# NBISweden/MrBayes

Hardware: AMD Instinct MI355X
Metric: site-pattern lnL (node-pattern conditional-likelihood) updates/sec (higher is better)
Workload: dtype f32

## Files before the change

### include/libhmsbeagle/beagle.h

```cpp
#ifndef MBAMD_LIBHMSBEAGLE_BEAGLE_H_
#define MBAMD_LIBHMSBEAGLE_BEAGLE_H_

#ifdef __cplusplus
extern "C" {
#endif

#define BEAGLE_DLLEXPORT __attribute__((visibility("default")))

enum BeagleReturnCodes {
    BEAGLE_SUCCESS                      =  0,
    BEAGLE_ERROR_GENERAL                = -1,
    BEAGLE_ERROR_OUT_OF_MEMORY          = -2,
    BEAGLE_ERROR_UNIDENTIFIED_EXCEPTION = -3,
    BEAGLE_ERROR_UNINITIALIZED_INSTANCE = -4,
    BEAGLE_ERROR_OUT_OF_RANGE           = -5,
    BEAGLE_ERROR_NO_RESOURCE            = -6,
    BEAGLE_ERROR_NO_IMPLEMENTATION      = -7,
    BEAGLE_ERROR_FLOATING_POINT         = -8
};

enum BeagleFlags {
    BEAGLE_FLAG_PRECISION_SINGLE    = 1 << 0,
    BEAGLE_FLAG_PRECISION_DOUBLE    = 1 << 1,
    BEAGLE_FLAG_COMPUTATION_SYNCH   = 1 << 2,
// ... 142 lines not shown
BEAGLE_DLLEXPORT int beagleWaitForPartials(int instance, const int* destinationPartials, int destinationPartialsCount);
BEAGLE_DLLEXPORT int beagleAccumulateScaleFactors(int instance, const int* scaleIndices, int count, int cumulativeScaleIndex);
BEAGLE_DLLEXPORT int beagleRemoveScaleFactors(int instance, const int* scaleIndices, int count, int cumulativeScaleIndex);
BEAGLE_DLLEXPORT int beagleResetScaleFactors(int instance, int cumulativeScaleIndex);
BEAGLE_DLLEXPORT int beagleCopyScaleFactors(int instance, int destScalingIndex, int srcScalingIndex);
BEAGLE_DLLEXPORT int beagleGetScaleFactors(int instance, int srcScalingIndex, double* outScaleFactors);

BEAGLE_DLLEXPORT int beagleCalculateRootLogLikelihoods(int instance, const int* bufferIndices,
                                                       const int* categoryWeightsIndices,
                                                       const int* stateFrequenciesIndices,
                                                       const int* cumulativeScaleIndices, int count,
                                                       double* outSumLogLikelihood);
BEAGLE_DLLEXPORT int beagleCalculateEdgeLogLikelihoods(int instance, const int* parentBufferIndices,
                                                       const int* childBufferIndices,
                                                       const int* probabilityIndices,
                                                       const int* firstDerivativeIndices,
                                                       const int* secondDerivativeIndices,
                                                       const int* categoryWeightsIndices,
                                                       const int* stateFrequenciesIndices,
                                                       const int* cumulativeScaleIndices, int count,
                                                       double* outSumLogLikelihood,
                                                       double* outSumFirstDerivative,
                                                       double* outSumSecondDerivative);
BEAGLE_DLLEXPORT int beagleGetSiteLogLikelihoods(int instance, double* outLogLikelihoods);
BEAGLE_DLLEXPORT int beagleGetSiteDerivatives(int instance, double* outFirstDerivatives, double* outSecondDerivatives);

BEAGLE_DLLEXPORT int beagleUpdatePrePartials(int instance, const BeagleOperation* operations, int operationCount,
                                             int cumulativeScaleIndex);
BEAGLE_DLLEXPORT int beagleSetDifferentialMatrix(int instance, int matrixIndex, const double* inMatrix);
BEAGLE_DLLEXPORT int beagleCalculateEdgeDerivatives(int instance, const int* postBufferIndices, const int* preBufferIndices,
                                                    const int* derivativeMatrixIndices, const int* categoryWeightsIndices,
                                                    int count, double* outDerivatives, double* outSumDerivatives,
                                                    double* outSumSquaredDerivatives);

BEAGLE_DLLEXPORT int beagleCalculateCrossProductDerivative(int instance, const int* postBufferIndices, const int* preBufferIndices,
                                                           const int* categoryRateIndices, const int* categoryWeightsIndices,
                                                           const double* edgeLengths, int count, double* outSumDerivatives,
                                                           double* outSumSquaredDerivatives);

BEAGLE_DLLEXPORT BeagleBenchmarkedResourceList* beagleGetBenchmarkedResourceList(
    int tipCount, int compactBufferCount, int stateCount, int patternCount, int categoryCount, int* resourceList,
    int resourceCount, long preferenceFlags, long requirementFlags, int eigenModelCount, int partitionCount,
    int calculateDerivatives, long benchmarkFlags);
BEAGLE_DLLEXPORT int beagleSetCPUThreadCount(int instance, int threadCount);
BEAGLE_DLLEXPORT int beagleSetPatternPartitions(int instance, int partitionCount, const int* inPatternPartitions);
BEAGLE_DLLEXPORT int beagleSetCategoryRatesWithIndex(int instance, int categoryRatesIndex, const double* inCategoryRates);
BEAGLE_DLLEXPORT int beagleUpdateTransitionMatricesWithMultipleModels(int instance, const int* eigenIndices,
                                                                      const int* categoryRateIndices,
                                                                      const int* probabilityIndices,
                                                                      const int* firstDerivativeIndices,
                                                                      const int* secondDerivativeIndices,
                                                                      const double* edgeLengths, int count);
BEAGLE_DLLEXPORT int beagleUpdatePartialsByPartition(int instance, const BeagleOperationByPartition* operations, int operationCount);
BEAGLE_DLLEXPORT int beagleAccumulateScaleFactorsByPartition(int instance, const int* scaleIndices, int count,
                                                             int cumulativeScaleIndex, int partitionIndex);
BEAGLE_DLLEXPORT int beagleRemoveScaleFactorsByPartition(int instance, const int* scaleIndices, int count,
                                                         int cumulativeScaleIndex, int partitionIndex);
BEAGLE_DLLEXPORT int beagleResetScaleFactorsByPartition(int instance, int cumulativeScaleIndex, int partitionIndex);
BEAGLE_DLLEXPORT int beagleCalculateRootLogLikelihoodsByPartition(int instance, const int* bufferIndices,
                                                                  const int* categoryWeightsIndices,
                                                                  const int* stateFrequenciesIndices,
                                                                  const int* cumulativeScaleIndices,
                                                                  const int* partitionIndices, int partitionCount, int count,
                                                                  double* outSumLogLikelihoodByPartition,
                                                                  double* outSumLogLikelihood);
BEAGLE_DLLEXPORT int beagleCalculateEdgeLogLikelihoodsByPartition(
    int instance, const int* parentBufferIndices, const int* childBufferIndices, const int* probabilityIndices,
    const int* firstDerivativeIndices, const int* secondDerivativeIndices, const int* categoryWeightsIndices,
    const int* stateFrequenciesIndices, const int* cumulativeScaleIndices, const int* partitionIndices, int partitionCount,
    int count, double* outSumLogLikelihoodByPartition, double* outSumLogLikelihood, double* outSumFirstDerivativeByPartition,
    double* outSumFirstDerivative, double* outSumSecondDerivativeByPartition, double* outSumSecondDerivative);

BEAGLE_DLLEXPORT int mbamdGetChildCount(int instance);
BEAGLE_DLLEXPORT int mbamdSynchronize(int instance);
BEAGLE_DLLEXPORT int mbamdGetScaleExponents(int instance, int srcScalingIndex, int* out);
BEAGLE_DLLEXPORT int mbamdSetRateMatrices(int instance, int firstEigenIndex, int count, const double* q, const double* pi, int mode);
BEAGLE_DLLEXPORT int mbamdSetRateMatricesFrom(int instance, int firstEigenIndex, int count, const double* q, const double* pi, int mode,
                                              int warmFirstEigenIndex);
BEAGLE_DLLEXPORT const char* mbamdGetLastError(void);
BEAGLE_DLLEXPORT int mbamdKernelTiming(int instance, int enable);
BEAGLE_DLLEXPORT int mbamdGetKernelTiming(int instance, double* outMilliseconds, long* outLaunches, int reset);
BEAGLE_DLLEXPORT int mbamdGetListCounts(int instance, long* out6);
BEAGLE_DLLEXPORT int mbamdGetWalkCounts(int instance, long* out2);
BEAGLE_DLLEXPORT int mbamdGetRecomputeCounts(int instance, long* out3);
BEAGLE_DLLEXPORT int mbamdGetSubtreeRecomputeCounts(int instance, long* out3);
BEAGLE_DLLEXPORT int mbamdGetStepTiming(int instance, double* outMilliseconds, long* outSteps, int reset);
BEAGLE_DLLEXPORT int mbamdSetKernelPath(int instance, int path);
BEAGLE_DLLEXPORT int mbamdSetDeferredResult(int instance, int enable);
BEAGLE_DLLEXPORT int mbamdWalkTrace(int instance, long long* out, int maxSteps, int* outSteps, int* outWaves);
BEAGLE_DLLEXPORT int mbamdFetchLogLikelihood(int instance, double* outSumLogLikelihood);
BEAGLE_DLLEXPORT int mbamdReduceLogLikelihood(int instance, double* deviceOut, void* waitingStream);
BEAGLE_DLLEXPORT int mbamdGetResourcePciBusId(int resource, char* out, int length);
BEAGLE_DLLEXPORT int mbamdGetInstanceDevices(int instance, int* outResources, int maxCount);

#ifdef __cplusplus
}
#endif
#endif
```

### mrbayes_amd/beagle.py

```python
from __future__ import annotations

import ctypes as C
import os
from typing import Optional, Sequence

import numpy as np

HERE = os.path.dirname(os.path.abspath(__file__))
DEFAULT_LIB = os.path.join(HERE, "libhmsbeagle.so")

BEAGLE_SUCCESS = 0
BEAGLE_ERROR_GENERAL = -1
BEAGLE_ERROR_OUT_OF_MEMORY = -2
BEAGLE_ERROR_UNINITIALIZED_INSTANCE = -4
BEAGLE_ERROR_OUT_OF_RANGE = -5
BEAGLE_ERROR_NO_RESOURCE = -6
BEAGLE_ERROR_NO_IMPLEMENTATION = -7
BEAGLE_ERROR_FLOATING_POINT = -8
BEAGLE_OP_NONE = -1

BEAGLE_FLAG_PRECISION_SINGLE = 1 << 0
BEAGLE_FLAG_PRECISION_DOUBLE = 1 << 1
BEAGLE_FLAG_EIGEN_REAL = 1 << 4
BEAGLE_FLAG_EIGEN_COMPLEX = 1 << 5
BEAGLE_FLAG_SCALING_ALWAYS = 1 << 8
BEAGLE_FLAG_SCALERS_LOG = 1 << 10
BEAGLE_FLAG_PROCESSOR_GPU = 1 << 16
BEAGLE_FLAG_SCALING_DYNAMIC = 1 << 25


class BeagleInstanceDetails(C.Structure):
    _fields_ = [("resourceNumber", C.c_int), ("resourceName", C.c_char_p), ("implName", C.c_char_p),
                ("implDescription", C.c_char_p), ("flags", C.c_long)]


class BeagleResource(C.Structure):
    _fields_ = [("name", C.c_char_p), ("description", C.c_char_p), ("supportFlags", C.c_long),
                ("requiredFlags", C.c_long)]


class BeagleResourceList(C.Structure):
    _fields_ = [("list", C.POINTER(BeagleResource)), ("length", C.c_int)]


class BeagleOperation(C.Structure):
    _fields_ = [("destinationPartials", C.c_int), ("destinationScaleWrite", C.c_int),
                ("destinationScaleRead", C.c_int), ("child1Partials", C.c_int),
                ("child1TransitionMatrix", C.c_int), ("child2Partials", C.c_int),
                ("child2TransitionMatrix", C.c_int)]


EXPORTS = [
    "beagleGetVersion", "beagleGetCitation", "beagleGetResourceList", "beagleCreateInstance",
    "beagleFinalizeInstance", "beagleFinalize", "beagleSetTipStates", "beagleSetTipPartials", "beagleSetPartials",
    "beagleGetPartials", "beagleSetEigenDecomposition", "beagleSetStateFrequencies", "beagleSetCategoryWeights",
    "beagleSetCategoryRates", "beagleSetPatternWeights", "beagleUpdateTransitionMatrices",
    "beagleSetTransitionMatrix", "beagleGetTransitionMatrix", "beagleConvolveTransitionMatrices", "beagleTransposeTransitionMatrices",
    "beagleSetTransitionMatrices", "beagleUpdatePartials", "beagleWaitForPartials",
    "beagleAccumulateScaleFactors", "beagleRemoveScaleFactors", "beagleResetScaleFactors", "beagleCopyScaleFactors",
    "beagleGetScaleFactors", "beagleCalculateRootLogLikelihoods", "beagleCalculateEdgeLogLikelihoods",
    "beagleGetSiteLogLikelihoods", "beagleGetSiteDerivatives", "beagleUpdatePrePartials", "beagleSetDifferentialMatrix",
    "beagleCalculateEdgeDerivatives", "beagleCalculateCrossProductDerivative", "mbamdSynchronize", "mbamdGetLastError", "mbamdKernelTiming",
    "mbamdGetKernelTiming", "mbamdGetListCounts", "mbamdGetWalkCounts", "mbamdGetRecomputeCounts", "mbamdGetSubtreeRecomputeCounts", "mbamdGetStepTiming", "mbamdUpdateFinalPartials", "mbamdGetScaledPartials", "mbamdSetKernelPath", "mbamdSetDeferredResult", "mbamdFetchLogLikelihood", "mbamdReduceLogLikelihood", "mbamdGetResourcePciBusId", "mbamdGetInstanceDevices",
    "mbamdGetScaleExponents", "mbamdGetChildCount", "mbamdSetRateMatrices", "mbamdSetRateMatricesFrom",
    "beagleGetBenchmarkedResourceList", "beagleSetCPUThreadCount", "beagleSetPatternPartitions",
    "beagleSetCategoryRatesWithIndex", "beagleUpdateTransitionMatricesWithMultipleModels", "beagleUpdatePartialsByPartition",
    "beagleAccumulateScaleFactorsByPartition", "beagleRemoveScaleFactorsByPartition", "beagleResetScaleFactorsByPartition",
    "beagleCalculateRootLogLikelihoodsByPartition", "beagleCalculateEdgeLogLikelihoodsByPartition",
]

_dp = C.POINTER(C.c_double)
_ip = C.POINTER(C.c_int)


class BeagleError(RuntimeError):
    def __init__(self, code: int, where: str, detail: str = ""):
        super().__init__("%s failed with code %d%s" % (where, code, (": " + detail) if detail else ""))
        self.code = code


def _d(a) -> np.ndarray:
    return np.ascontiguousarray(a, dtype=np.float64)


def _i(a) -> np.ndarray:
    return np.ascontiguousarray(a, dtype=np.int32)


def _opt_i(a) -> Optional[np.ndarray]:
    return None if a is None else _i(a)


def _ptr(a: Optional[np.ndarray]):
    return None if a is None else a.ctypes.data_as(_ip)


class BeagleLibrary:

    def __init__(self, path: Optional[str] = None):
        path = path or os.environ.get("MBAMD_LIBRARY") or DEFAULT_LIB
        if not os.path.exists(path):
            raise FileNotFoundError(
                "%s not found: build the HIP engine first (python -m mrbayes_amd.build). "
                "There is no CPU implementation to fall back to." % path)
        self.path = path
        self.lib = C.CDLL(path)
        for name in EXPORTS:
            if not hasattr(self.lib, name):
                raise AttributeError("%s does not export %s" % (path, name))
        L = self.lib
        L.beagleGetVersion.restype = C.c_char_p
        L.beagleGetCitation.restype = C.c_char_p
        L.mbamdGetLastError.restype = C.c_char_p
        L.beagleGetResourceList.restype = C.POINTER(BeagleResourceList)
        L.beagleCreateInstance.argtypes = [C.c_int] * 9 + [_ip, C.c_int, C.c_long, C.c_long,
                                                          C.POINTER(BeagleInstanceDetails)]
        L.beagleSetTipStates.argtypes = [C.c_int, C.c_int, _ip]
        L.beagleSetTipPartials.argtypes = [C.c_int, C.c_int, _dp]
        L.beagleSetPartials.argtypes = [C.c_int, C.c_int, _dp]
        L.beagleGetPartials.argtypes = [C.c_int, C.c_int, C.c_int, _dp]
        L.beagleSetEigenDecomposition.argtypes = [C.c_int, C.c_int, _dp, _dp, _dp]
        L.beagleSetStateFrequencies.argtypes = [C.c_int, C.c_int, _dp]
        L.beagleSetCategoryWeights.argtypes = [C.c_int, C.c_int, _dp]
        L.beagleSetCategoryRates.argtypes = [C.c_int, _dp]
        L.beagleSetPatternWeights.argtypes = [C.c_int, _dp]
        L.beagleUpdateTransitionMatrices.argtypes = [C.c_int, C.c_int, _ip, _ip, _ip, _dp, C.c_int]
        L.beagleSetTransitionMatrix.argtypes = [C.c_int, C.c_int, _dp, C.c_double]
        L.beagleGetTransitionMatrix.argtypes = [C.c_int, C.c_int, _dp]
        L.beagleConvolveTransitionMatrices.argtypes = [C.c_int, _ip, _ip, _ip, C.c_int]
        L.beagleTransposeTransitionMatrices.argtypes = [C.c_int, _ip, _ip, C.c_int]
        L.beagleSetTransitionMatrices.argtypes = [C.c_int, _ip, _dp, _dp, C.c_int]
        L.beagleUpdatePartials.argtypes = [C.c_int, C.POINTER(BeagleOperation), C.c_int, C.c_int]
        L.beagleWaitForPartials.argtypes = [C.c_int, _ip, C.c_int]
        L.beagleAccumulateScaleFactors.argtypes = [C.c_int, _ip, C.c_int, C.c_int]
        L.beagleRemoveScaleFactors.argtypes = [C.c_int, _ip, C.c_int, C.c_int]
        L.beagleResetScaleFactors.argtypes = [C.c_int, C.c_int]
        L.beagleCopyScaleFactors.argtypes = [C.c_int, C.c_int, C.c_int]
        L.beagleGetScaleFactors.argtypes = [C.c_int, C.c_int, _dp]
        L.beagleCalculateRootLogLikelihoods.argtypes = [C.c_int, _ip, _ip, _ip, _ip, C.c_int, _dp]
        L.beagleCalculateEdgeLogLikelihoods.argtypes = [C.c_int, _ip, _ip, _ip, _ip, _ip, _ip, _ip, _ip, C.c_int,
                                                        _dp, _dp, _dp]
        L.beagleGetSiteLogLikelihoods.argtypes = [C.c_int, _dp]
        L.beagleGetSiteDerivatives.argtypes = [C.c_int, _dp, _dp]
        L.beagleUpdatePrePartials.argtypes = [C.c_int, C.POINTER(BeagleOperation), C.c_int, C.c_int]
        L.beagleSetDifferentialMatrix.argtypes = [C.c_int, C.c_int, _dp]
        L.beagleCalculateEdgeDerivatives.argtypes = [C.c_int, _ip, _ip, _ip, _ip, C.c_int, _dp, _dp, _dp]
        L.beagleCalculateCrossProductDerivative.argtypes = [C.c_int, _ip, _ip, _ip, _ip, _dp, C.c_int, _dp, _dp]
        L.mbamdGetKernelTiming.argtypes = [C.c_int, _dp, C.POINTER(C.c_long), C.c_int]
        L.mbamdGetListCounts.argtypes = [C.c_int, C.POINTER(C.c_long)]
        L.mbamdGetWalkCounts.argtypes = [C.c_int, C.POINTER(C.c_long)]
        L.mbamdGetRecomputeCounts.argtypes = [C.c_int, C.POINTER(C.c_long)]
        L.mbamdGetSubtreeRecomputeCounts.argtypes = [C.c_int, C.POINTER(C.c_long)]
        L.mbamdGetStepTiming.argtypes = [C.c_int, _dp, C.POINTER(C.c_long), C.c_int]
        L.mbamdUpdateFinalPartials.argtypes = [C.c_int, C.c_void_p, C.c_int]
        L.mbamdGetScaledPartials.argtypes = [C.c_int, C.c_int, C.c_int, C.POINTER(C.c_float), C.POINTER(C.c_float)]
        L.mbamdFetchLogLikelihood.argtypes = [C.c_int, _dp]
        L.mbamdReduceLogLikelihood.argtypes = [C.c_int, C.c_void_p, C.c_void_p]
        L.mbamdGetResourcePciBusId.argtypes = [C.c_int, C.c_char_p, C.c_int]
        L.mbamdGetInstanceDevices.argtypes = [C.c_int, _ip, C.c_int]

    def version(self) -> str:
        return self.lib.beagleGetVersion().decode()

    def last_error(self) -> str:
        return self.lib.mbamdGetLastError().decode()

    def pci_bus_id(self, resource: int) -> str:
        buf = C.create_string_buffer(64)
        rc = self.lib.mbamdGetResourcePciBusId(resource, buf, 64)
        if rc != 0:
            raise BeagleError(rc, "mbamdGetResourcePciBusId", self.last_error())
        return buf.value.decode()

    def resources(self):
        rl = self.lib.beagleGetResourceList().contents
        return [(rl.list[i].name.decode(), rl.list[i].description.decode(), rl.list[i].supportFlags)
                for i in range(rl.length)]


_default: Optional[BeagleLibrary] = None


def library(path: Optional[str] = None) -> BeagleLibrary:
    global _default
    if path is not None:
        return BeagleLibrary(path)
    if _default is None:
        _default = BeagleLibrary()
    return _default


class BeagleInstance:

    def __init__(self, lib: BeagleLibrary, tip_count, partials_buffer_count, compact_buffer_count, state_count,
                 pattern_count, eigen_buffer_count, matrix_buffer_count, category_count, scale_buffer_count,
                 resource: Optional[int] = None, preference_flags=0, requirement_flags=0):
        self._L = lib
        self.lib = lib.lib
        self.details = BeagleInstanceDetails()
        rl = None
        rc = 0
        if resource is not None:
            arr = (C.c_int * 1)(resource)
            rl, rc = C.cast(arr, _ip), 1
        self.id = self.lib.beagleCreateInstance(tip_count, partials_buffer_count, compact_buffer_count, state_count,
                                                pattern_count, eigen_buffer_count, matrix_buffer_count,
                                                category_count, scale_buffer_count, rl, rc, preference_flags,
                                                requirement_flags, C.byref(self.details))
        if self.id < 0:
            raise BeagleError(self.id, "beagleCreateInstance", lib.last_error())
        self.state_count, self.pattern_count, self.category_count = state_count, pattern_count, category_count

    def _chk(self, code: int, where: str, allow=()):
        if code != BEAGLE_SUCCESS and code not in allow:
            raise BeagleError(code, where, self._L.last_error())
        return code

    def finalize(self):
        if self.id >= 0:
            self.lib.beagleFinalizeInstance(self.id)
            self.id = -1

    def __del__(self):
        try:
            self.finalize()
        except Exception:
            pass

    def set_tip_states(self, tip, states):
        a = _i(states)
        self._chk(self.lib.beagleSetTipStates(self.id, tip, a.ctypes.data_as(_ip)), "beagleSetTipStates")

    def set_tip_partials(self, tip, partials):
# ... 203 lines not shown
        self._chk(self.lib.beagleUpdateTransitionMatricesWithMultipleModels(
            self.id, g.ctypes.data_as(_ip), r.ctypes.data_as(_ip), p.ctypes.data_as(_ip), _ptr(d1), _ptr(d2), e.ctypes.data_as(_dp), len(p)),
            "beagleUpdateTransitionMatricesWithMultipleModels")

    def update_partials_by_partition(self, operations):
        a = _i(operations).reshape(-1, 9)
        self._chk(self.lib.beagleUpdatePartialsByPartition(self.id, a.ctypes.data_as(C.c_void_p), a.shape[0]),
                  "beagleUpdatePartialsByPartition")

    def reset_scale_factors_by_partition(self, cum, partition):
        self._chk(self.lib.beagleResetScaleFactorsByPartition(self.id, cum, partition), "beagleResetScaleFactorsByPartition")

    def accumulate_scale_factors_by_partition(self, idx, cum, partition):
        a = _i(idx)
        self._chk(self.lib.beagleAccumulateScaleFactorsByPartition(self.id, a.ctypes.data_as(_ip), len(a), cum, partition),
                  "beagleAccumulateScaleFactorsByPartition")

    def remove_scale_factors_by_partition(self, idx, cum, partition):
        a = _i(idx)
        self._chk(self.lib.beagleRemoveScaleFactorsByPartition(self.id, a.ctypes.data_as(_ip), len(a), cum, partition),
                  "beagleRemoveScaleFactorsByPartition")

    def calculate_edge_log_likelihoods_by_partition(self, parents, children, probs, weights, freqs, cums, partitions, count):
        p, ch, pr, w, f, c, pt = _i(parents), _i(children), _i(probs), _i(weights), _i(freqs), _i(cums), _i(partitions)
        by = np.zeros(len(pt))
        out = C.c_double(0.0)
        rc = self.lib.beagleCalculateEdgeLogLikelihoodsByPartition(
            self.id, p.ctypes.data_as(_ip), ch.ctypes.data_as(_ip), pr.ctypes.data_as(_ip), None, None, w.ctypes.data_as(_ip),
            f.ctypes.data_as(_ip), c.ctypes.data_as(_ip), pt.ctypes.data_as(_ip), len(pt), count, by.ctypes.data_as(_dp),
            C.byref(out), None, None, None, None)
        self._chk(rc, "beagleCalculateEdgeLogLikelihoodsByPartition", allow=(BEAGLE_ERROR_FLOATING_POINT,))
        return rc, by, out.value

    def calculate_edge_derivatives_by_partition(self, parents, children, probs, first, second, weights, freqs, cums, partitions):
        p, ch, pr, w, f, c, pt = _i(parents), _i(children), _i(probs), _i(weights), _i(freqs), _i(cums), _i(partitions)
        d1, d2 = _opt_i(first), _opt_i(second)
        by = [np.zeros(len(pt)) for _ in range(3)]
        tot = [C.c_double(0.0) for _ in range(3)]
        rc = self.lib.beagleCalculateEdgeLogLikelihoodsByPartition(
            self.id, p.ctypes.data_as(_ip), ch.ctypes.data_as(_ip), pr.ctypes.data_as(_ip), _ptr(d1), _ptr(d2), w.ctypes.data_as(_ip),
            f.ctypes.data_as(_ip), c.ctypes.data_as(_ip), pt.ctypes.data_as(_ip), len(pt), 1, by[0].ctypes.data_as(_dp), C.byref(tot[0]),
            by[1].ctypes.data_as(_dp) if d1 is not None else None, C.byref(tot[1]) if d1 is not None else None,
            by[2].ctypes.data_as(_dp) if d2 is not None else None, C.byref(tot[2]) if d2 is not None else None)
        self._chk(rc, "beagleCalculateEdgeLogLikelihoodsByPartition", allow=(BEAGLE_ERROR_FLOATING_POINT,))
        return (rc, (by[0], tot[0].value), (by[1], tot[1].value) if d1 is not None else None,
                (by[2], tot[2].value) if d2 is not None else None)

    def calculate_root_log_likelihoods_by_partition(self, buffers, weights, freqs, cums, partitions, count):
        b, w, f, c, pt = _i(buffers), _i(weights), _i(freqs), _i(cums), _i(partitions)
        by = np.zeros(len(pt))
        out = C.c_double(0.0)
        rc = self.lib.beagleCalculateRootLogLikelihoodsByPartition(
            self.id, b.ctypes.data_as(_ip), w.ctypes.data_as(_ip), f.ctypes.data_as(_ip), c.ctypes.data_as(_ip),
            pt.ctypes.data_as(_ip), len(pt), count, by.ctypes.data_as(_dp), C.byref(out))
        self._chk(rc, "beagleCalculateRootLogLikelihoodsByPartition", allow=(BEAGLE_ERROR_FLOATING_POINT,))
        return rc, by, out.value

    def get_site_log_likelihoods(self) -> np.ndarray:
        out = np.empty(self.pattern_count)
        self._chk(self.lib.beagleGetSiteLogLikelihoods(self.id, out.ctypes.data_as(_dp)), "beagleGetSiteLogLikelihoods")
        return out

    def synchronize(self):
        self._chk(self.lib.mbamdSynchronize(self.id), "mbamdSynchronize")

    def kernel_timing(self, enable: bool):
        self._chk(self.lib.mbamdKernelTiming(self.id, 1 if enable else 0), "mbamdKernelTiming")

    def get_kernel_timing(self, reset=True):
        ms, n = C.c_double(0.0), C.c_long(0)
        self._chk(self.lib.mbamdGetKernelTiming(self.id, C.byref(ms), C.byref(n), 1 if reset else 0), "mbamdGetKernelTiming")
        return ms.value, n.value

    def get_list_counts(self):
        out = (C.c_long * 6)()
        self._chk(self.lib.mbamdGetListCounts(self.id, out), "mbamdGetListCounts")
        return tuple(int(v) for v in out)

    def get_walk_counts(self):
        out = (C.c_long * 2)()
        self._chk(self.lib.mbamdGetWalkCounts(self.id, out), "mbamdGetWalkCounts")
        return tuple(int(v) for v in out)

    def get_recompute_counts(self):
        out = (C.c_long * 3)()
        self._chk(self.lib.mbamdGetRecomputeCounts(self.id, out), "mbamdGetRecomputeCounts")
        return tuple(int(v) for v in out)

    def get_subtree_recompute_counts(self):
        out = (C.c_long * 3)()
        self._chk(self.lib.mbamdGetSubtreeRecomputeCounts(self.id, out), "mbamdGetSubtreeRecomputeCounts")
        return tuple(int(v) for v in out)

    def update_final_partials(self, operations):
        a = _i(operations).reshape(-1, 5)
        self._chk(self.lib.mbamdUpdateFinalPartials(self.id, a.ctypes.data_as(C.c_void_p), a.shape[0]), "mbamdUpdateFinalPartials")

    def get_scaled_partials(self, idx, cumulative_scale_index=BEAGLE_OP_NONE):
        out = np.empty((self.category_count, self.pattern_count, self.state_count), dtype=np.float32)
        ln = np.empty(self.pattern_count, dtype=np.float32)
        self._chk(self.lib.mbamdGetScaledPartials(self.id, idx, cumulative_scale_index, out.ctypes.data_as(C.POINTER(C.c_float)),
                                                  ln.ctypes.data_as(C.POINTER(C.c_float))), "mbamdGetScaledPartials")
        return out, ln

    def get_step_timing(self, reset=True):
        ms, n = C.c_double(0.0), C.c_long(0)
        self._chk(self.lib.mbamdGetStepTiming(self.id, C.byref(ms), C.byref(n), 1 if reset else 0), "mbamdGetStepTiming")
        return ms.value, n.value

    def set_deferred_result(self, enable: bool):
        self._chk(self.lib.mbamdSetDeferredResult(self.id, 1 if enable else 0), "mbamdSetDeferredResult")

    def reduce_log_likelihood(self, device_ptr, waiting_stream=0):
        self._chk(self.lib.mbamdReduceLogLikelihood(self.id, C.c_void_p(device_ptr), C.c_void_p(waiting_stream)), "mbamdReduceLogLikelihood")

    def devices(self):
        out = (C.c_int * 64)()
        n = self.lib.mbamdGetInstanceDevices(self.id, C.cast(out, _ip), 64)
        return [int(out[i]) for i in range(min(n, 64))]

    def fetch_log_likelihood(self):
        out = C.c_double(0.0)
        rc = self.lib.mbamdFetchLogLikelihood(self.id, C.byref(out))
        self._chk(rc, "mbamdFetchLogLikelihood", allow=(BEAGLE_ERROR_FLOATING_POINT,))
        return rc, out.value
```

### mrbayes_amd/csrc/mbamd_engine.cpp

```cpp
#include <mutex>
#include <memory>

#include "mbamd_host.h"
#include "libhmsbeagle/mbamd_parsimony.h"
#include "mbamd_parsimony.h"
#include "mbamd_f32.h"
#include "mbamd_f64.h"

namespace mbamd {

static std::mutex g_mutex;

static BeagleResourceList g_resources = {nullptr, 0};
static std::vector<BeagleResource> g_resourceVec;
static std::vector<std::string> g_resourceNames, g_resourceDescs;
static const long kSupport = BEAGLE_FLAG_PRECISION_SINGLE | BEAGLE_FLAG_COMPUTATION_SYNCH | BEAGLE_FLAG_EIGEN_REAL |
                             BEAGLE_FLAG_SCALING_MANUAL | BEAGLE_FLAG_SCALING_ALWAYS | BEAGLE_FLAG_SCALING_DYNAMIC |
                             BEAGLE_FLAG_SCALERS_LOG | BEAGLE_FLAG_VECTOR_NONE | BEAGLE_FLAG_THREADING_NONE |
                             BEAGLE_FLAG_PROCESSOR_GPU | BEAGLE_FLAG_INVEVEC_STANDARD | BEAGLE_FLAG_FRAMEWORK_HIP;

static void buildResources()
{
    if (g_resources.list) return;
    int n = 0;
// ... 928 lines not shown
        if (crc) return crc;
        for (size_t e = 0; e < n; ++e) { sum[e] += part[e]; sq[e] += partSq[e]; }
        return BEAGLE_SUCCESS;
    });
    if (rc) return rc;
    if (outSumDerivatives) std::copy(sum.begin(), sum.end(), outSumDerivatives);
    if (outSumSquaredDerivatives) std::copy(sq.begin(), sq.end(), outSumSquaredDerivatives);
    return BEAGLE_SUCCESS;
}

int beagleCalculateCrossProductDerivative(int instance, const int* postBufferIndices, const int* preBufferIndices, const int* categoryRateIndices,
                                          const int* categoryWeightsIndices, const double* edgeLengths, int count, double* outSumDerivatives,
                                          double* outSumSquaredDerivatives)
{
    StatTimer st_(ST_LNL);
    GET_INSTANCE(instance);
    API_TRACE("beagleCalculateCrossProductDerivative(count=%d)", count);
    const char* const who = "beagleCalculateCrossProductDerivative";
    if (h->partitionCount > 1) return fail(BEAGLE_ERROR_NO_IMPLEMENTATION, who, "not on a multi-partition instance");
    if (outSumSquaredDerivatives) return fail(BEAGLE_ERROR_NO_IMPLEMENTATION, who, "outSumSquaredDerivatives must be NULL (a per-pattern square is an S x S matrix per pattern)");
    if (count < 0 || !outSumDerivatives ||
        (count > 0 && (!postBufferIndices || !preBufferIndices || !categoryRateIndices || !categoryWeightsIndices || !edgeLengths)))
        return fail(BEAGLE_ERROR_OUT_OF_RANGE, who, "null array");
    if (h->f64)
        return h->f64->crossProducts(postBufferIndices, preBufferIndices, categoryRateIndices, categoryWeightsIndices, edgeLengths, count, outSumDerivatives);
    const size_t SS = (size_t) h->dim.stateCount * h->dim.stateCount;
    std::vector<double> sum(SS, 0.0), part(SS);
    const int rc = each_engine(h, true, [&](Instance* c, const Handle::Span&) -> int {
        const int crc = c->crossProducts(postBufferIndices, preBufferIndices, categoryRateIndices, categoryWeightsIndices, edgeLengths, count, part.data());
        if (crc) return crc;
        for (size_t ij = 0; ij < SS; ++ij) sum[ij] += part[ij];
        return BEAGLE_SUCCESS;
    });
    if (rc) return rc;
    std::copy(sum.begin(), sum.end(), outSumDerivatives);
    return BEAGLE_SUCCESS;
}

int mbamdSynchronize(int instance)
{
    GET_INSTANCE(instance);
    return synchronize(h);
}
int mbamdKernelTiming(int instance, int enable)
{
    GET_INSTANCE(instance);
    if (h->f64) return BEAGLE_SUCCESS;
    EACH_ENGINE(false, (c->setTiming(enable != 0), BEAGLE_SUCCESS));
}
int mbamdGetKernelTiming(int instance, double* outMilliseconds, long* outLaunches, int reset)
{
    GET_INSTANCE(instance);
    double ms = 0.0;
    long launches = 0;
    const int rc = h->f64 ? h->f64->kernelTiming(&ms, &launches, reset) : each_engine(h, false, [&](Instance* c, const Handle::Span&) {
        double m = 0.0;
        const int trc = c->kernelTiming(&m, &launches, reset);
        ms = std::max(ms, m);
        return trc;
    });
    if (rc) return rc;
    if (outMilliseconds) *outMilliseconds = ms;
    if (outLaunches) *outLaunches = launches;
    return BEAGLE_SUCCESS;
}
int mbamdGetListCounts(int instance, long* out6)
{
    GET_INSTANCE(instance);
    if (!out6) return fail(BEAGLE_ERROR_OUT_OF_RANGE, "mbamdGetListCounts: null output");
    for (int i = 0; i < 6; ++i) out6[i] = 0;
    if (!in) return BEAGLE_SUCCESS;
    in->listCounts(out6);
    return BEAGLE_SUCCESS;
}
int mbamdGetWalkCounts(int instance, long* out2)
{
    GET_INSTANCE(instance);
    if (!out2) return fail(BEAGLE_ERROR_OUT_OF_RANGE, "mbamdGetWalkCounts: null output");
    out2[0] = out2[1] = 0;
    if (!in) return BEAGLE_SUCCESS;
    in->walkCounts(out2);
    return BEAGLE_SUCCESS;
}
int mbamdGetRecomputeCounts(int instance, long* out3)
{
    GET_INSTANCE_NOFLUSH(instance);
    if (!out3) return fail(BEAGLE_ERROR_OUT_OF_RANGE, "mbamdGetRecomputeCounts: null output");
    out3[0] = out3[1] = out3[2] = 0;
    if (h->f64) return BEAGLE_SUCCESS;
    EACH_ENGINE(false, (c->recomputeCounts(out3), BEAGLE_SUCCESS));
}
int mbamdGetSubtreeRecomputeCounts(int instance, long* out3)
{
    GET_INSTANCE_NOFLUSH(instance);
    if (!out3) return fail(BEAGLE_ERROR_OUT_OF_RANGE, "mbamdGetSubtreeRecomputeCounts: null output");
    out3[0] = out3[1] = out3[2] = 0;
    if (h->f64) return BEAGLE_SUCCESS;
    EACH_ENGINE(false, (c->subtreeRecomputeCounts(out3), BEAGLE_SUCCESS));
}
int mbamdGetStepTiming(int instance, double* outMilliseconds, long* outSteps, int reset)
{
    GET_INSTANCE(instance);
    if (h->f64) return fail(BEAGLE_ERROR_NO_IMPLEMENTATION, "mbamdGetStepTiming: not on a double-precision instance");
    double ms = 0.0;
    long steps = 0;
    const int rc = each_engine(h, false, [&](Instance* c, const Handle::Span&) {
        double m = 0.0;
        long st = 0;
        const int trc = c->stepTiming(&m, &st, reset);
        ms = std::max(ms, m);
        steps = std::max(steps, st);
        return trc;
    });
    if (rc) return rc;
    if (outMilliseconds) *outMilliseconds = ms;
    if (outSteps) *outSteps = steps;
    return BEAGLE_SUCCESS;
}
int mbamdSetKernelPath(int instance, int path)
{
    GET_INSTANCE(instance);
    if (h->f64) return BEAGLE_SUCCESS;
    if (path < 0 || path > 3) return fail(BEAGLE_ERROR_OUT_OF_RANGE, "mbamdSetKernelPath");
    return BEAGLE_SUCCESS;
}
int mbamdWalkTrace(int instance, long long* out, int maxSteps, int* outSteps, int* outWaves)
{
    GET_INSTANCE(instance);
    if (h->f64) return fail(BEAGLE_ERROR_NO_IMPLEMENTATION, "mbamdWalkTrace: not on a double-precision instance");
    if (!in) return fail(BEAGLE_ERROR_GENERAL, "set MBAMD_WALK_TRACE before creating the instance");
    return in->walkTrace(out, maxSteps, outSteps, outWaves);
}
int mbamdGetChildCount(int instance)
{
    GET_INSTANCE_NOFLUSH(instance);
    if (h->f64) return h->f64->childCount();
    return h->children.empty() ? 1 : (int) h->children.size();
}
int mbamdSetDeferredResult(int instance, int enable)
{
    GET_INSTANCE(instance);
    if (h->f64) return enable ? fail(BEAGLE_ERROR_NO_IMPLEMENTATION, "mbamdSetDeferredResult: not on a double-precision instance") : BEAGLE_SUCCESS;
    if (!in) return enable ? fail(BEAGLE_ERROR_NO_IMPLEMENTATION, "mbamdSetDeferredResult: not on a partitioned / sharded instance") : BEAGLE_SUCCESS;
    in->setDeferredResult(enable != 0);
    return BEAGLE_SUCCESS;
}
int mbamdReduceLogLikelihood(int instance, double* deviceOut, void* waitingStream)
{
    GET_INSTANCE(instance);
    if (!in) return fail(BEAGLE_ERROR_NO_IMPLEMENTATION, "mbamdReduceLogLikelihood: plain single-precision instances only");
    return in->reduceResult(deviceOut, waitingStream);
}
int mbamdGetResourcePciBusId(int resource, char* out, int length)
{
    if (out == nullptr || length < 2) return fail(BEAGLE_ERROR_OUT_OF_RANGE, "mbamdGetResourcePciBusId: buffer");
    int n = 0;
    if (hipGetDeviceCount(&n) != hipSuccess || resource < 0 || resource >= n) return fail(BEAGLE_ERROR_OUT_OF_RANGE, "mbamdGetResourcePciBusId: resource");
    HIP_TRY(hipDeviceGetPCIBusId(out, length, resource));
    return BEAGLE_SUCCESS;
}
int mbamdGetInstanceDevices(int instance, int* outResources, int maxCount)
{
    GET_INSTANCE_NOFLUSH(instance);
    if (h->children.empty()) { if (outResources && maxCount > 0) outResources[0] = h->device; return 1; }
    int n = 0;
    for (const Handle::Child& c : h->children) { if (outResources && n < maxCount) outResources[n] = c.in->device; ++n; }
// ... 142 lines not shown
```

### mrbayes_amd/csrc/mbamd_f32.h

```cpp
#ifndef MBAMD_F32_H_
#define MBAMD_F32_H_

#include <cmath>
#include <cstdlib>
#include <memory>
#include <unordered_map>

#include "mbamd_host.h"
#include "mbamd_kernels.h"
#include "mbamd_reports.h"
#include "libhmsbeagle/mbamd_reports.h"
#include "mbamd_walk4_host.h"
#include "mbamd_kernels_mfma.h"
#include "mbamd_derivatives.h"
#include "mbamd_preorder.h"
#include "mbamd_crossproducts.h"
#include "mbamd_matrix_products.h"

namespace mbamd {


static inline bool wg_compiled(int S) { return (S >= 2 && S <= 10 && S != 4) || S == 16 || S == 20 || S == 40 || (S >= 60 && S <= 63); }
#if !defined(MBAMD_WG_DEPTH61)
#define MBAMD_WG_DEPTH61 1
#endif
#define MBAMD_WG_DISPATCH(S, FN, ...)                                   \
    switch (S) {                                                        \
        case 2: FN<2, 8, 1, 2>(__VA_ARGS__); break;                     \
        case 3: FN<3, 8, 1, 2>(__VA_ARGS__); break;                     \
        case 5: FN<5, 8, 1, 2>(__VA_ARGS__); break;                     \
        case 6: FN<6, 8, 1, 2>(__VA_ARGS__); break;                     \
        case 7: FN<7, 8, 1, 2>(__VA_ARGS__); break;                     \
        case 8: FN<8, 8, 1, 2>(__VA_ARGS__); break;                     \
        case 9: FN<9, 8, 1, 2>(__VA_ARGS__); break;                     \
        case 10: FN<10, 8, 1, 2>(__VA_ARGS__); break;                   \
        case 16: FN<16, 8, 1, 2>(__VA_ARGS__); break;                   \
        case 20: FN<20, 8, 1, 2>(__VA_ARGS__); break;                   \
        case 40: FN<40, 4, 1, 1>(__VA_ARGS__); break;                   \
        case 60: FN<60, 4, 2, MBAMD_WG_DEPTH61>(__VA_ARGS__); break;    \
        case 61: FN<61, 4, 2, MBAMD_WG_DEPTH61>(__VA_ARGS__); break;    \
        case 62: FN<62, 4, 2, MBAMD_WG_DEPTH61>(__VA_ARGS__); break;    \
        default: FN<63, 4, 2, MBAMD_WG_DEPTH61>(__VA_ARGS__); break;    \
    }

template <int SC_, int WMAX_, int CH_, int DEPTH_>
static void raise_walkg_lds(int maxLds)
{
    if (hipFuncSetAttribute((const void*) k_walkg<SC_, WMAX_, CH_, DEPTH_>, hipFuncAttributeMaxDynamicSharedMemorySize, maxLds) != hipSuccess ||
        hipFuncSetAttribute((const void*) k_walkg<SC_, WMAX_, CH_, DEPTH_, WalkGArgsInline>, hipFuncAttributeMaxDynamicSharedMemorySize, maxLds) != hipSuccess)
        (void) hipGetLastError();
}

#define MBAMD_W4_UNSTORED_TIPS_DEFAULT 4
struct Walk4Recipe {
    int nops = 0;
    struct Op { int c1, c2, mode; bool in1, in2; } op[MBAMD_W4_UNSTORED_TIPS_MAX - 1];
    bool usesTip(int tip) const
    {
        for (int j = 0; j < nops; ++j) if ((!op[j].in1 && op[j].c1 == tip) || (!op[j].in2 && op[j].c2 == tip)) return true;
        return false;
    }
};

struct Plan {
    std::vector<int> key;
    uint64_t hash = 0, lastUse = 0;
    uint64_t lastLaunch = 0;
    PartialsOp* d_table = nullptr;
    size_t cap = 0;
    struct Segment {
        size_t first; int W, entries, nslots, tail = 2;
        bool plain = false, peel = false;
    };
    std::vector<Segment> segments;
    std::vector<Walk4Entry> inlineProg;
    struct Unstored { int entry, dst; Walk4Recipe r; int inner[MBAMD_W4_UNSTORED_TIPS_MAX - 2]; };
    std::vector<Unstored> unstoredSubtrees;
    size_t sideFirst = 0; int sideCount = 0;
    bool path = false;
    bool forked = false;
    bool pathG = false;
    int lists = 1;
    std::vector<int> start;
    bool anyScale = false;
    bool narrow = false;
    std::vector<std::pair<int, int>> chains;
    std::vector<std::pair<int, int>> spineChains;
    int tipTip = 0;
    int serialFrom = 0;
    std::vector<int> bufsRead, bufsWritten, scalesUsed;
};

struct PathStep {
    bool start, join;
    bool chainTip, sibTip;
    int arm;
    int dst, chain, sib;
    int mchain, msib;
    int scaleMode, scaleIdx;
};

struct Instance;
static int new_engine(std::unique_ptr<Instance>& out, const Dims& d, int patternCount, int dev, const Switches& sw);

struct Instance {
    Instance() = default;
    Instance(const Instance&) = delete;
    Instance& operator=(const Instance&) = delete;
    ~Instance();
    int device = 0;
    const char* implName() const;
    void printStats(int id) const;
    int synchronize() { HIP_TRY(hipStreamSynchronize(stream)); return BEAGLE_SUCCESS; }
    int setTipStates(int tip, const int* states);
    int importPartials(int idx, const double* in, bool hasCategories);
    int getPartials(int idx, double* out);
    int setPatternWeights(const double* w, int count) { return upload(d_pweights, w, sizeof(double) * count); }
    int setEigen(int idx, const double* U, const double* Ui, const double* lam);
    int setRateMatrices(int first, int count, const double* q, const double* pi, int mode, int warmFirst = -1);
    int setRates(int index, const double* r);
    int updateMatrices(int eigenIndex, const int* probIdx, const double* lengths, int count, int rateSet = 0,
                       const int* d1Idx = nullptr, const int* d2Idx = nullptr);
    int setMatrix(int idx, const double* in);
    int getMatrix(int idx, double* out);
    int convolveMatrices(const int* first, const int* second, const int* result, int count);
    int transposeMatrices(const int* input, const int* result, int count);
    int setMatrices(const int* idx, const double* in, int count);
    int updatePartials(const BeagleOperation* ops, int n, int cumIdx);
    int flushPending(bool keepPath = false);
    int resetScale(int idx, bool mayWait = false);
    int copyScale(int dst, int src);
    int accumulateScale(const int* idx, int n, int cumIdx, int sign, bool afterReset = false);
    int runDeferredReset() { const int idx = deferredReset; deferredReset = -1; return idx < 0 ? BEAGLE_SUCCESS : resetScale(idx); }
    int getScaleExponents(int idx, int* out);
    int integrate(const int* parent, const int* child, const int* prob, const int* wIdx, const int* fIdx,
                  const int* cumIdx, int count, double* out, bool launchOnly = false);
    int fetchResult(double* out);
    void setDeferredResult(bool on) { deferred = on; }
    int reduceResult(double* deviceOut, void* waitingStream);
    bool hasSites() const { return haveSite; }
    int getSites(double* out);
    int edgeDerivatives(int parent, int child, int prob, int d1, int d2, int wIdx, int fIdx, int cumIdx, double out3[3]);
    bool hasDerivatives() const { return derivValid; }
    const double* siteDerivatives(int order) const { return h_deriv + (size_t) order * Ppad; }
    int updatePrePartials(const BeagleOperation* ops, int n, int cumIdx);
    int edgeGradient(const int* post, const int* pre, const int* dmat, const int* wIdx, int count, double* sites, size_t siteStride,
                     double* sums, double* sumsSq);
    int crossProducts(const int* post, const int* pre, const int* rateIdx, const int* wIdx, const double* lengths, int count, double* out);
    int finalPass(const MbamdFinalOperation* ops, int count);
    int getScaledPartials(int idx, int cumIdx, float* out, float* outLn);
    void setTiming(bool on) { timing = on; }
    int kernelTiming(double* ms, long* launches, int reset);
    int stepTiming(double* ms, long* steps, int reset);
    void listCounts(long out6[6]) const { const long c[6] = {listsTotal, listsPath, forkedPaths, fusedPaths, listsWalked, opsWalked}; std::copy(c, c + 6, out6); }
    void walkCounts(long out2[2]) const { out2[0] = walksPlain; out2[1] = walksGeneric; }
    int walkTrace(long long* out, int maxSteps, int* outSteps, int* outWaves);
    void recomputeCounts(long out3[3]) const { out3[0] += leftUnstored; out3[1] += materialised; out3[2] += materialiseLaunches; }
    void subtreeRecomputeCounts(long out3[3]) const { out3[0] += leftUnstoredSub; out3[1] += materialisedSub; out3[2] += materialiseLaunchesSub; }

private:
    friend int new_engine(std::unique_ptr<Instance>&, const Dims&, int, int, const Switches&);
    hipStream_t stream{};
    int tipCount = 0, nBuffers = 0, S = 0, SP = 0, P = 0, Ppad = 0, nEigen = 0, nMatrices = 0, K = 0, nScale = 0;
    bool complexEigen = false;
    bool s4 = false;
    bool wg = false;
    bool noWalkG = false;
    bool arena() const { return s4 || wg; }
    bool mfma = false;
    int walkWaves = 1, lastWalkSteps = 0;
    Walk4Builder w4;
    std::unordered_map<uint64_t, Walk4Template> w4templates;
    uint64_t scheduleHits = 0, scheduleMisses = 0;
    std::vector<Walk4Op> w4ops;
    std::vector<int> w4key, w4writer, w4segList;
    std::vector<char> w4written, w4segRead, w4segWritten, w4segScale;
    std::vector<Walk4Entry> w4table;
    int8_t* arenaExp = nullptr;
    unsigned estride = 0;
    std::vector<int32_t*> wideScale;
    std::vector<char> scaleState;
    int lastWalkW = 0, lastWalkSlots = 0, lastWalkEntries = 0, lastWalkPhases = 0;
    bool walkCumFresh = false;
    typedef Walk4Recipe Recipe;
    std::vector<char> unstored;
    std::vector<Recipe> recipes;
    int nUnstored = 0;
    float* d_snap = nullptr;
    Plan* snapPlan = nullptr;
    void* d_storeProg = nullptr;     size_t storeProgCap = 0;
    std::vector<int> storeList;
    std::vector<Walk4Entry> storeProg;
    long leftUnstored = 0, materialised = 0, materialiseLaunches = 0;
    long leftUnstoredSub = 0, materialisedSub = 0, materialiseLaunchesSub = 0;
    int unstoredTips() const { return std::max(2, std::min(MBAMD_W4_UNSTORED_TIPS_MAX, sw.unstoredTips.value_or(MBAMD_W4_UNSTORED_TIPS_DEFAULT))); }
    std::vector<int> w4subTips, w4subOps, w4entryOf;
    int leaveUnstored(const Plan& plan);
    int flushSnapshot();
    int ensureStored(const int* bufs, int n);
    int ensureStoredSubtrees();
    int ensureStored(int a, int b = -1) { const int v[2] = {a, b}; return nUnstored ? ensureStored(v, 2) : BEAGLE_SUCCESS; }
    int storeUsersOfTip(int tip);
    void dropRecipe(int idx) { if (nUnstored && unstored[(size_t) idx]) { unstored[(size_t) idx] = 0; --nUnstored; } }
    std::vector<BeagleOperation> wgOps;
    std::vector<int> wgListStart, wgListCum;
    int32_t* wgCum[MBAMD_WG_MAXLISTS] = {nullptr, nullptr, nullptr, nullptr};
    int wgFresh = 0;
    uint8_t* arenaTipStates = nullptr;
    unsigned long wgTileBytes = 0;
    unsigned wgTipTileBytes = 0;
    size_t wgTabFloats = 0;
public:
    bool hasPending(bool path = true) const { return !pending.empty() || !wgListCum.empty() || (path && heldPath != nullptr); }
    bool hasWork(bool path = true) const { return hasPending(path) || !pendingJobs.empty(); }
private:
    Plan* heldPath = nullptr;
    int32_t* heldPathCum = nullptr;
    bool heldPathFresh = false;
    int heldPathDst = -1;
    int runHeldPath();
    int integratePath4(const int* child, const int* prob, const int* wIdx, const int* fIdx, const int* cumIdx);
    int updatePartialsG(const BeagleOperation* ops, int n, int cumIdx);
    int flushWalkG();
    int runWalkG(const Plan& plan);
    int checkOperation(const BeagleOperation& b, const std::vector<char>& written, const char*& what) const;
    std::vector<PathStep> pathSteps;
    bool recognisePath(const BeagleOperation* ops, int n, int L, bool& forked);
    Walk4Entry pathEntry(const PathStep& p, uint32_t pbuf, uint32_t tipb, uint32_t mbuf, int scratchRow) const;
    void pathPlan(Plan& plan, int entries, bool forked);
    bool buildPath4(Plan& plan, const BeagleOperation* ops, int n);
    bool buildPathG(Plan& plan, const BeagleOperation* ops, int n, const std::vector<int>& starts, int nl);
    Walk4Args walk4Args() const;
    WalkGArgs walkGArgs() const;
    int prepareCumulative(int idx, bool& fresh);
    void postResultFlag();
    bool scaleOpsIndependentOfPending(const int* idx, int n, int cumIdx) const;
    uint64_t launchClock = 0, syncedClock = 0;
    uint64_t flagClock = 0;
    uint32_t siteSeq = 0, seenSeq = 0;
    HostMirror h_freqs, h_weights;
    long long* d_trace = nullptr;

    int NT = 0, T = 0;
    size_t partialsFloats = 0, matrixFloats = 0, eigenDoubles = 0;

    std::vector<float*> partials;
    std::vector<uint8_t*> tipStates;
    std::vector<int32_t*> scale;
    std::vector<char> valid;
    float* arenaPartials = nullptr;
    uint64_t* arenaTips = nullptr;
    BlockGeom geom{64, 64, 64};
    float* matrices = nullptr;
    double *d_eigen = nullptr, *d_freqs = nullptr, *d_weights = nullptr, *d_rates = nullptr, *d_pweights = nullptr;
    double *d_site = nullptr;
    double* h_site = nullptr;
    double* h_site_dev = nullptr;
    bool siteToHost = false, siteOnHost = false;
    int nblocks = 0;
    double* h_deriv = nullptr;
    double* h_deriv_dev = nullptr;
    bool derivValid = false;
    std::vector<char> preOrder;
    void clearPreOrder(int idx) { if (idx >= 0 && idx < (int) preOrder.size()) preOrder[idx] = 0; }
    LnlOperands lastLnl;
// ... 69 lines not shown
    void armSums(bool launchOnly) { sumsArmed = !pendingResult && !deferred && !launchOnly && wait.arm(h_sums, (size_t) nblocks); }

    bool timing = false;
    std::vector<std::pair<hipEvent_t, hipEvent_t>> events;
    double timedMs = 0.0;
    long timedLaunches = 0, pendingLaunches = 0;
    hipEvent_t spanEv0{};
    bool spanOpen = false;
    std::vector<std::pair<hipEvent_t, hipEvent_t>> spans;
    double spanMs = 0.0;
    long spanCount = 0;
    int spanBegin()
    {
        if (!timing || spanOpen) return BEAGLE_SUCCESS;
        HIP_TRY(hipEventCreate(&spanEv0));
        HIP_TRY(hipEventRecord(spanEv0, stream));
        spanOpen = true;
        return BEAGLE_SUCCESS;
    }
    int spanEnd()
    {
        if (!spanOpen) return BEAGLE_SUCCESS;
        hipEvent_t e1{};
        HIP_TRY(hipEventCreate(&e1));
        HIP_TRY(hipEventRecord(e1, stream));
        spans.emplace_back(spanEv0, e1);
        spanOpen = false;
        if (spans.size() > 4096) {
            HIP_TRY(hipStreamSynchronize(stream));
            spanFold();
        }
        return BEAGLE_SUCCESS;
    }
    int spanFold()
    {
        for (auto& ev : spans) {
            float t = 0.0f;
            if (hipEventElapsedTime(&t, ev.first, ev.second) == hipSuccess) { spanMs += t; ++spanCount; }
            (void) hipEventDestroy(ev.first);
            (void) hipEventDestroy(ev.second);
        }
        spans.clear();
        return BEAGLE_SUCCESS;
    }
    int launchesBegin(hipEvent_t& ev0, hipEvent_t& ev1)
    {
        { int src = spanBegin(); if (src) return src; }
        if (!timing) return BEAGLE_SUCCESS;
        HIP_TRY(hipEventCreate(&ev0));
        HIP_TRY(hipEventCreate(&ev1));
        HIP_TRY(hipEventRecord(ev0, stream));
        return BEAGLE_SUCCESS;
    }
    int launchesEnd(hipEvent_t ev0, hipEvent_t ev1)
    {
        if (!timing) return BEAGLE_SUCCESS;
        HIP_TRY(hipEventRecord(ev1, stream));
        events.emplace_back(ev0, ev1);
        return BEAGLE_SUCCESS;
    }
    int eventsFold()
    {
        for (auto& ev : events) {
            float t = 0.0f;
            HIP_TRY(hipEventElapsedTime(&t, ev.first, ev.second));
            timedMs += t;
            (void) hipEventDestroy(ev.first);
            (void) hipEventDestroy(ev.second);
        }
        events.clear();
        return BEAGLE_SUCCESS;
    }

    bool deferred = false, pendingResult = false;
    hipEvent_t reduceEvent{};
    std::vector<int32_t*> finalExpOf;
    std::unordered_map<int, int32_t*> finalExpOwn;

    std::vector<std::pair<Plan*, int>> pending;
    std::vector<Plan*> plans;
    uint64_t planClock = 0;
    int layoutEpoch = 0;
    long planHits = 0, planMisses = 0, fusedPaths = 0, heldPaths = 0, forkedPaths = 0, listsTotal = 0, listsPath = 0, opsWalked = 0, listsWalked = 0;
    long walksPlain = 0, walksGeneric = 0;

    int grow(void** p, size_t* cap, size_t bytes) { return grow_device(stream, p, cap, bytes, std::max(bytes, *cap * 2)); }

    int upload(void* dst, const void* src, size_t bytes)
    {
        if (bytes == 0) return BEAGLE_SUCCESS;
        if (bytes > stage.capacity() / 2) {
            HIP_TRY(hipStreamSynchronize(stream));
            HIP_TRY(hipMemcpy(dst, src, bytes, hipMemcpyHostToDevice));
            return BEAGLE_SUCCESS;
        }
        if (bytes <= ((size_t) 256 << 10) && bytes % 4 == 0 && (reinterpret_cast<uintptr_t>(dst) & 3u) == 0) return ringCopy(dst, src, bytes);
        size_t off = 0;
        int rc = stage.put(src, bytes, stream, &off);
        if (rc) return rc;
        HIP_TRY(hipMemcpyAsync(dst, stage.host(off), bytes, hipMemcpyHostToDevice, stream));
        return BEAGLE_SUCCESS;
    }
    int ringCopy(void* dst, const void* src, size_t bytes);

public:
    int setFreqs(int idx, const double* f) { return h_freqs.send((size_t) nEigen * S, (size_t) idx * S, f, (size_t) S, [&] { return upload(d_freqs + (size_t) idx * S, f, sizeof(double) * S); }); }
    int setWeights(int idx, const double* w) { return h_weights.send((size_t) nEigen * K, (size_t) idx * K, w, (size_t) K, [&] { return upload(d_weights + (size_t) idx * K, w, sizeof(double) * K); }); }
private:

    int stageDirect(const void* src, size_t bytes, const void** devPtr)
    {
        if (((bytes + 63) & ~(size_t) 63) > stage.capacity() / 2) return fail(BEAGLE_ERROR_OUT_OF_MEMORY, "staging ring too small");
        size_t off = 0;
        int rc = stage.put(src, bytes, stream, &off);
        if (rc) return rc;
        *devPtr = stage.dev(off);
        return BEAGLE_SUCCESS;
    }

    int ensurePartials(int idx)
    {
        if (partials[idx]) return BEAGLE_SUCCESS;
        if (arena()) return fail(BEAGLE_ERROR_GENERAL, "partials arena not initialised");
        float* p = nullptr;
        HIP_TRY(hipMalloc(&p, partialsFloats * sizeof(float)));
        HIP_TRY(hipMemsetAsync(p, 0, partialsFloats * sizeof(float), stream));
        partials[idx] = p;
        return BEAGLE_SUCCESS;
    }
    int ensureScale(int idx)
    {
        if (scale[idx]) return BEAGLE_SUCCESS;
        if (arena()) return fail(BEAGLE_ERROR_GENERAL, "exponent arena not initialised");
        int32_t* p = nullptr;
        HIP_TRY(hipMalloc(&p, (size_t) Ppad * sizeof(int32_t)));
        HIP_TRY(hipMemsetAsync(p, 0, (size_t) Ppad * sizeof(int32_t), stream));
        scale[idx] = p;
        return BEAGLE_SUCCESS;
    }
    float* matrixPtr(int idx) const { return matrices + (size_t) idx * matrixFloats; }

    int create(const Dims& dim, int patternCount, int dev, const Switches& switches);

    int configureWalk();
    void wgGeometry(int lists, int& W, int& slots) const;
    int setTipMasks(int tip, const std::vector<uint8_t>& masks);
    std::vector<int> eigenWarm;
    std::vector<char> eigenShield;
    int updatePartials4(const BeagleOperation* ops, int n, int cumIdx);
    int buildWalk(Plan& plan, const BeagleOperation* ops, int n, const int* listOf = nullptr, bool perList = false);
    int ensureWide(int idx);
    int accumulate4(const int* idx, int n, int cumIdx, int sign);
    int deferredReset = -1;
    int checkIntegrate(const int* parent, const int* child, const int* prob, const int* wIdx, const int* fIdx, const int* cumIdx, int count);
    int integrate4(const int* parent, const int* child, const int* prob, const int* wIdx, const int* fIdx,
                   const int* cumIdx, int count);
    int integrateLevels(const int* parent, const int* child, const int* prob, const int* wIdx, const int* fIdx,
                        const int* cumIdx, int count);
    int buildGeneric(Plan& plan, std::vector<PartialsOp>& dev, const std::vector<int>& dstIdx, const std::vector<int>& c1Idx,
                     const std::vector<int>& c2Idx);
    int runWalk(const Plan& plan, int32_t* cum);
    int runGeneric(const Plan& plan, int32_t* cum);
    Plan* cachedPlan(const int* key, size_t nints, bool& build);
    int planBuilt(Plan& plan, int rc);
    int planTable(Plan& plan, const void* table, size_t bytes);
    int timedRun(const Plan& plan, int32_t* cum);
// ... 122 lines not shown
        wgTileBytes = (unsigned long) (nBuffers + 1) * K * tb;
        wgTipTileBytes = (unsigned) nBuffers * MBAMD_WG_TW;
        estride = (unsigned) (scale.size() + MBAMD_WG_SCRATCH_ROWS) * K * 64;
        const size_t pBytes = nt * wgTileBytes, tBytes = nt * wgTipTileBytes, eBytes = nb * (size_t) estride;
        HIP_TRY(hipMalloc(&arenaPartials, pBytes));
        HIP_TRY(hipMalloc(&arenaTipStates, tBytes));
        HIP_TRY(hipMalloc(&arenaExp, eBytes));
        HIP_TRY(hipMemsetAsync(arenaPartials, 0, pBytes, stream));
        HIP_TRY(hipMemsetAsync(arenaTipStates, S, tBytes, stream));
        HIP_TRY(hipMemsetAsync(arenaExp, 0, eBytes, stream));
        wideScale.assign(scale.size(), nullptr);
        scaleState.assign(scale.size(), 0);
        if (sw.verbose)
            std::fprintf(stderr, "[mbamd] arenas: partials +%zu, tips +%zu, exponents +%zu bytes\n", pBytes, tBytes, eBytes);
        for (int i = 0; i < nBuffers; ++i) partials[i] = arenaPartials + (size_t) i * K * tb / 4;
    }

    HIP_TRY(hipMalloc(&matrices, std::max<size_t>(1, (size_t) nMatrices * matrixFloats) * sizeof(float)));
    HIP_TRY(hipMemsetAsync(matrices, 0, std::max<size_t>(1, (size_t) nMatrices * matrixFloats) * sizeof(float), stream));
    if (wg && nMatrices > 0) {
        const int total = nMatrices * K * S;
        MBAMD_LAUNCH(k_wg_init_tables, (unsigned) ((total + 255) / 256), 256, 0, stream, matrices, matrixFloats, wgTabFloats, S, K, total);
        HIP_TRY(hipGetLastError());
    }
    HIP_TRY(hipMalloc(&d_eigen, std::max<size_t>(1, (size_t) nEigen * eigenDoubles) * sizeof(double)));
    if (complexEigen) HIP_TRY(hipMemsetAsync(d_eigen, 0, std::max<size_t>(1, (size_t) nEigen * eigenDoubles) * sizeof(double), stream));
    HIP_TRY(hipMalloc(&d_freqs, std::max<size_t>(1, (size_t) nEigen * S) * sizeof(double)));
    HIP_TRY(hipMalloc(&d_weights, std::max<size_t>(1, (size_t) nEigen * K) * sizeof(double)));
    HIP_TRY(hipMalloc(&d_rates, (size_t) K * sizeof(double)));
    HIP_TRY(hipMalloc(&d_pweights, (size_t) Ppad * sizeof(double)));
    HIP_TRY(hipMalloc(&d_site, (size_t) Ppad * sizeof(double)));
    nblocks = Ppad / 64;
    if (!s4 && S >= 8) nblocks = Ppad / 32;
    if (wg) nblocks = Ppad / MBAMD_INTEGRATE_WG_PATTERNS;
    HIP_TRY(hipHostMalloc(&h_sums, (size_t) nblocks * sizeof(double), hipHostMallocDefault));
    HIP_TRY(hipHostGetDevicePointer((void**) &h_sums_dev, h_sums, 0));
    wait.create(!sw.noPoll);
    { int rc = stage.create((size_t) 8 << 20, 64); if (rc) return rc; }

    std::vector<double> ones(std::max(Ppad, K), 1.0);
    HIP_TRY(hipMemcpy(d_rates, ones.data(), (size_t) K * sizeof(double), hipMemcpyHostToDevice));
    std::vector<double> pw(Ppad, 0.0);
    std::fill(pw.begin(), pw.begin() + P, 1.0);
    HIP_TRY(hipMemcpy(d_pweights, pw.data(), (size_t) Ppad * sizeof(double), hipMemcpyHostToDevice));
    std::vector<double> w((size_t) std::max(1, nEigen) * K, 1.0 / K);
    HIP_TRY(hipMemcpy(d_weights, w.data(), (size_t) nEigen * K * sizeof(double), hipMemcpyHostToDevice));
    HIP_TRY(hipStreamSynchronize(stream));
    return BEAGLE_SUCCESS;
}

inline Instance::~Instance()
{
    (void) hipSetDevice(device);
    (void) hipStreamSynchronize(stream);
    if (arena()) {
        void* arenas[] = {arenaPartials, arenaTips, arenaTipStates, arenaExp};
        for (void* a : arenas) if (a) (void) hipFree(a);
        for (int32_t* w : wideScale) if (w) (void) hipFree(w);
    } else {
        for (float* p : partials) if (p) (void) hipFree(p);
        for (uint8_t* p : tipStates) if (p) (void) hipFree(p);
        for (int32_t* p : scale) if (p) (void) hipFree(p);
    }
    pending.clear();
    wgOps.clear(); wgListStart.clear(); wgListCum.clear();
    for (Plan* pl : plans) { if (pl->d_table) (void) hipFree(pl->d_table); delete pl; }
    plans.clear();
    void* bufs[] = {matrices, d_eigen, d_freqs, d_weights, d_rates, d_pweights, d_site,
                    d_ev, d_tmp, d_trace, d_q, d_preTable, d_snap, d_storeProg};
    for (void* b : bufs) if (b) (void) hipFree(b);
    if (h_sums) (void) hipHostFree(h_sums);
    wait.destroy();
    if (h_site) (void) hipHostFree(h_site);
    if (h_deriv) (void) hipHostFree(h_deriv);
    stage.destroy();
    for (auto& ev : events) { (void) hipEventDestroy(ev.first); (void) hipEventDestroy(ev.second); }
    for (auto& ev : spans) { (void) hipEventDestroy(ev.first); (void) hipEventDestroy(ev.second); }
    if (spanOpen) (void) hipEventDestroy(spanEv0);
    if (reduceEvent) (void) hipEventDestroy(reduceEvent);
    for (auto& kv : finalExpOwn) if (kv.second) (void) hipFree(kv.second);
    (void) hipStreamDestroy(stream);
}

inline int Instance::configureWalk()
{
    int numCU = 256;
    hipDeviceProp_t prop;
    if (hipGetDeviceProperties(&prop, device) == hipSuccess && prop.multiProcessorCount > 0) numCU = prop.multiProcessorCount;
    const int maxLds = 160 * 1024;
    if (s4 && (hipFuncSetAttribute((const void*) k_walk4_t<Walk4Args>, hipFuncAttributeMaxDynamicSharedMemorySize, maxLds) != hipSuccess ||
               hipFuncSetAttribute((const void*) k_walk4_t<Walk4Args, true>, hipFuncAttributeMaxDynamicSharedMemorySize, maxLds) != hipSuccess ||
               hipFuncSetAttribute((const void*) k_walk4_t<Walk4ArgsInline>, hipFuncAttributeMaxDynamicSharedMemorySize, maxLds) != hipSuccess))
        (void) hipGetLastError();
    if (wg) {
        const unsigned slotBytes = wg_block_bytes(S);
        MBAMD_WG_DISPATCH(S, raise_walkg_lds, maxLds);
        wgGeometry(1, w4.maxW, w4.maxSlots);
        w4.maxSlots1 = w4.maxSlots;
        if (!sw.walkWaves && !sw.maxLdsSlots) {
            const long wgsG = (long) (Ppad / MBAMD_WG_TW) * K;
            const int perCUG = (int) std::max(1L, (wgsG + numCU - 1) / numCU);
            w4.maxSlots1 = std::max(w4.maxSlots, std::min(24, (int) (((160 * 1024) / std::min(perCUG, 32) - 64 - MBAMD_WG_STAGE) / (int) slotBytes)));
        }
        w4.memSlots = false;
        w4.leadNops = MBAMD_WG_LEAD; w4.unroll = 3; w4.tailNops = MBAMD_WG_TAIL;
        w4.prefetchDistance = 0;
        if (sw.walkSmallPhase) w4.smallPhase = std::max(1, *sw.walkSmallPhase);
        if (sw.verbose) std::fprintf(stderr, "[mbamd] tree walk (%d states): %ld workgroups, up to %d waves x %d slots of %u bytes\n",
                                     S, (long) (Ppad / MBAMD_WG_TW) * K, w4.maxW, w4.maxSlots, slotBytes);
        return BEAGLE_SUCCESS;
    }
    const long wgs = (long) (Ppad / 64) * K;
    const int perCU = (int) std::max(1L, (wgs + numCU - 1) / numCU);
    const int ldsPerWG = (160 * 1024) / std::min(perCU, 32) - 64;
    auto slotsFor = [&](int W) { return (ldsPerWG / W - MBAMD_W4_STAGE) / 1024; };
    int W = (int) std::max(1L, std::min((long) MBAMD_W4_MAXW, (14L * numCU + wgs / 2) / wgs));
    while (W > 1 && slotsFor(W) < 7) --W;
    if (sw.walkWaves) W = std::max(1, std::min(MBAMD_W4_MAXW, *sw.walkWaves));
    int slots = std::max(3, std::min(48, slotsFor(W)));
    if (sw.maxLdsSlots) slots = std::max(3, std::min(150 / W, *sw.maxLdsSlots));
    w4.maxW = W;
    w4.maxSlots = slots;
    w4.maxSlots1 = sw.maxLdsSlots ? slots : std::max(slots, std::min(40, slotsFor(1)));
    if (sw.walkPrefetch) w4.prefetchDistance = std::max(0, *sw.walkPrefetch);
    w4.forward = true;
    w4.safeWaits = sw.walkSafe;
    if (sw.walkSmallPhase) w4.smallPhase = std::max(1, *sw.walkSmallPhase);
    if (sw.verbose) std::fprintf(stderr, "[mbamd] tree walk: %ld workgroups (%d per CU), up to %d waves x %d slots\n", wgs, perCU, W, slots);
    return BEAGLE_SUCCESS;
}

inline void Instance::wgGeometry(int lists, int& W, int& slots) const
{
    int numCU = 256;
    hipDeviceProp_t prop;
    if (hipGetDeviceProperties(&prop, device) == hipSuccess && prop.multiProcessorCount > 0) numCU = prop.multiProcessorCount;
    const int maxW = S > 32 ? 4 : 8, wavesPerCU = S > 32 ? 6 : 12;
    const int slotBytes = (int) wg_block_bytes(S);
    const long wgs = (long) (Ppad / MBAMD_WG_TW) * K * lists;
    const int perCU = (int) std::max(1L, (wgs + numCU - 1) / numCU);
    const int ldsPerWG = (160 * 1024) / std::min(perCU, 32) - 64;
    auto slotsFor = [&](int w) { return (ldsPerWG / w - MBAMD_WG_STAGE) / slotBytes; };
    long want = std::max(1L, std::min((long) maxW, ((long) wavesPerCU * numCU + wgs / 2) / wgs));
    W = 1;
    while (W * 2 <= want) W *= 2;
    while (W > 1 && slotsFor(W) < 4) W /= 2;
    if (sw.walkWaves) W = std::max(1, std::min(maxW, *sw.walkWaves));
    slots = std::max(3, std::min(24, slotsFor(W)));
    if (sw.maxLdsSlots) slots = std::max(1, std::min((160 * 1024 / W - MBAMD_WG_STAGE) / slotBytes, *sw.maxLdsSlots));
}

inline int Instance::setTipMasks(int tip, const std::vector<uint8_t>& h)
{
    const size_t nb = (size_t) Ppad / 64;
    std::vector<uint64_t> planes(nb * 4, 0);
    for (int c = 0; c < Ppad; ++c)
        for (int i = 0; i < 4; ++i)
            if (h[c] >> i & 1u) planes[(size_t) (c >> 6) * 4 + i] |= (uint64_t) 1 << (c & 63);
    if (nUnstored) {
        const int src = storeUsersOfTip(tip);
        if (src) return src;
        dropRecipe(tip);
    }
    HIP_TRY(hipStreamSynchronize(stream));
    HIP_TRY(hipMemcpy2D(arenaTips + (size_t) tip * 4, (size_t) geom.tstride * 8, planes.data(), 32, 32, nb, hipMemcpyHostToDevice));
    if (!tipStates[tip]) layoutEpoch++;
    tipStates[tip] = reinterpret_cast<uint8_t*>(arenaTips + (size_t) tip * 4);
    return BEAGLE_SUCCESS;
}

inline int Instance::setTipStates(int tip, const int* states)
{
    if (tip < 0 || tip >= nBuffers) return fail(BEAGLE_ERROR_OUT_OF_RANGE, "beagleSetTipStates: tip index");
    clearPreOrder(tip);
    std::vector<uint8_t> h(Ppad, (uint8_t) S);
    for (int c = 0; c < P; ++c) h[c] = (uint8_t) ((states[c] < 0 || states[c] >= S) ? S : states[c]);
    if (s4) {
        for (int c = 0; c < Ppad; ++c) h[c] = (uint8_t) (h[c] >= 4 ? 0xF : 1u << h[c]);
        return setTipMasks(tip, h);
    }
    if (wg) {
        HIP_TRY(hipStreamSynchronize(stream));
        HIP_TRY(hipMemcpy2D(arenaTipStates + (size_t) tip * MBAMD_WG_TW, (size_t) wgTipTileBytes, h.data(), MBAMD_WG_TW, MBAMD_WG_TW, (size_t) Ppad / MBAMD_WG_TW, hipMemcpyHostToDevice));
        if (!tipStates[tip]) layoutEpoch++;
        tipStates[tip] = arenaTipStates + (size_t) tip * MBAMD_WG_TW;
        return BEAGLE_SUCCESS;
    }
    if (!tipStates[tip]) { HIP_TRY(hipMalloc(&tipStates[tip], (size_t) Ppad)); layoutEpoch++; }
    return upload(tipStates[tip], h.data(), (size_t) Ppad);
}

inline int Instance::importPartials(int idx, const double* in, bool hasCategories)
{
    if (idx < 0 || idx >= nBuffers) return fail(BEAGLE_ERROR_OUT_OF_RANGE, "partials buffer index");
    if (idx < (int) finalExpOf.size()) finalExpOf[idx] = nullptr;
    clearPreOrder(idx);
    if (s4 && !hasCategories) {
        std::vector<uint8_t> h(Ppad, 0xF);
        bool binary = true;
        for (int c = 0; c < P && binary; ++c) {
            unsigned m = 0;
            for (int i = 0; i < 4; ++i) {
                const double v = in[(size_t) c * 4 + i];
                if (v == 1.0) m |= 1u << i;
                else if (v != 0.0) binary = false;
            }
            h[c] = (uint8_t) m;
        }
        if (binary) return setTipMasks(idx, h);
    }
// ... 672 lines not shown
    scaleState[idx] = 2;
    return BEAGLE_SUCCESS;
}

inline int Instance::updatePartials4(const BeagleOperation* ops, int n, int cumIdx)
{
    if (heldPath) { int prc = runHeldPath(); if (prc) return prc; }
    if (snapPlan) { int src = flushSnapshot(); if (src) return src; }
    if (nUnstored) {
        std::vector<int>& ext = w4segList;
        std::vector<char>& written = w4written;
        ext.clear();
        written.assign((size_t) nBuffers, 0);
        for (int o = 0; o < n; ++o) {
            for (const int c : {ops[o].child1Partials, ops[o].child2Partials})
                if (c >= 0 && c < nBuffers && unstored[(size_t) c] && !written[(size_t) c]) ext.push_back(c);
            if (ops[o].destinationPartials >= 0 && ops[o].destinationPartials < nBuffers) written[(size_t) ops[o].destinationPartials] = 1;
        }
        if (!ext.empty()) { int src = ensureStored(ext.data(), (int) ext.size()); if (src) return src; }
    }
    int32_t* cumPtr = nullptr;
    walkCumFresh = false;
    if (cumIdx != BEAGLE_OP_NONE) {
        int rc = prepareCumulative(cumIdx, walkCumFresh);
        if (rc) return rc;
        cumPtr = wideScale[cumIdx];
    }
    bool build;
    Plan* plan = cachedPlan(reinterpret_cast<const int*>(ops), (size_t) n * 7, build);
    if (build) {
        int rc = flushMatrices();
        if (rc == BEAGLE_SUCCESS) {
            StatTimer st_(ST_PLAN);
            plan->path = plan->forked = false;
            plan->unstoredSubtrees.clear();
            rc = buildPath4(*plan, ops, n) ? BEAGLE_SUCCESS : buildWalk(*plan, ops, n);
        }
        if (planBuilt(*plan, rc)) return rc;
    }
    for (int o = 0; o < n; ++o) {
        valid[ops[o].destinationPartials] = 1;
        dropRecipe(ops[o].destinationPartials);
        if (ops[o].destinationScaleWrite != BEAGLE_OP_NONE) scaleState[ops[o].destinationScaleWrite] = 1;
    }
    int mrc = flushMatrices();
    if (mrc) return mrc;
    listsTotal++;
    if (plan->path) { listsPath++; if (plan->forked) forkedPaths++; }
    else { listsWalked++; opsWalked += n; }
    if (plan->path && !sw.noFusePath && K <= 8 && plan->inlineProg.size() <= MBAMD_W4_INLINE) {
        heldPath = plan;
        heldPaths++;
        heldPathCum = cumPtr;
        heldPathFresh = walkCumFresh;
        heldPathDst = ops[n - 1].destinationPartials;
        return BEAGLE_SUCCESS;
    }
    return timedRun(*plan, cumPtr);
}

inline int Instance::buildWalk(Plan& plan, const BeagleOperation* ops, int n, const int* listOf, bool perList)
{
    const int scratchScale = (int) scale.size();
    std::vector<int>& segList = w4segList;
    segList.clear();
    std::vector<char>& written = w4written;
    written.assign((size_t) nBuffers, 0);
    w4table.clear();
    plan.segments.clear();
    plan.unstoredSubtrees.clear();
    std::vector<Walk4Op>& seg = w4ops;
    seg.clear();
    std::vector<char>&segRead = w4segRead, &segWritten = w4segWritten, &segScale = w4segScale;
    segRead.assign((size_t) nBuffers, 0); segWritten.assign((size_t) nBuffers, 0); segScale.assign(scale.size() + 1, 0);
    if (w4writer.size() < (size_t) nBuffers) w4writer.assign((size_t) nBuffers, -1);
    int reloads = 0, externals = 0, phases = 0;
    auto flushSegment = [&]() -> int {
        if (seg.empty()) return BEAGLE_SUCCESS;
        std::vector<int>& key = w4key;
        key.clear();
        key.reserve(seg.size() * 3 + 4);
        key.push_back((int) seg.size()); key.push_back(w4.maxW); key.push_back(w4.maxSlots + 256 * w4.maxSlots1);
        key.push_back(w4.prefetchDistance * 2 + (w4.safeWaits ? 1 : 0));
        {
            std::vector<int>& writer = w4writer;
            constexpr int RO = MBAMD_W4_UNSTORED_TIPS_MAX - 1;
            w4subTips.assign(wg ? 0 : seg.size(), 0);
            w4subOps.assign(wg ? 0 : seg.size() * RO, -1);
            for (size_t o = 0; o < seg.size() && !wg; ++o) {
                const Walk4Op& op = seg[o];
                const int w1 = op.tip1 ? -1 : writer[op.c1], w2 = op.tip2 ? -1 : writer[op.c2];
                const int t1 = op.tip1 ? 1 : (w1 >= 0 ? w4subTips[(size_t) w1] : 0), t2 = op.tip2 ? 1 : (w2 >= 0 ? w4subTips[(size_t) w2] : 0);
                if (t1 && t2 && t1 + t2 <= MBAMD_W4_UNSTORED_TIPS_MAX && (op.tip1 || op.tip2 || op.c1 != op.c2)) {
                    w4subTips[o] = t1 + t2;
                    int below = 0, *mine = &w4subOps[o * RO];
                    for (const int w : {std::min(w1, w2), std::max(w1, w2)})
                        for (int j = 0; w >= 0 && j < RO && w4subOps[(size_t) w * RO + j] >= 0; ++j) mine[below++] = w4subOps[(size_t) w * RO + j];
                    mine[below] = (int) o;
                }
                writer[op.dst] = (int) o;
            }
            for (size_t o = 0; o < seg.size() && !wg; ++o) writer[seg[o].dst] = -1;
            for (size_t o = 0; o < seg.size(); ++o) {
                key.push_back(seg[o].tip1 ? -1 : writer[seg[o].c1]);
                key.push_back(seg[o].tip2 ? -1 : writer[seg[o].c2]);
                key.push_back((int) seg[o].tip1 | ((int) seg[o].tip2 << 1) | ((!seg[o].tip1 && !seg[o].tip2 && seg[o].c1 == seg[o].c2) ? 4 : 0) |
                              ((seg[o].scaleWrite < 0 && seg[o].scaleRead >= 0) ? 8 : 0));
                writer[seg[o].dst] = (int) o;
            }
            for (size_t o = 0; o < seg.size(); ++o) writer[seg[o].dst] = -1;
        }
        const uint64_t kh = fnv1a(key.data(), key.size());
        auto it = w4templates.find(kh);
        if (it == w4templates.end() || it->second.key != key) {
            scheduleMisses++;
            if (w4templates.size() >= 8192) w4templates.clear();
            Walk4Template& t = w4templates[kh];
            bool ok = w4.build(seg, t);
            if (!ok) {
                Walk4Builder plain = w4;
                plain.prefetchDistance = 0;
                ok = plain.build(seg, t);
                if (!ok) { plain.maxW = 1; ok = plain.build(seg, t); }
            }
            if (!ok) { w4templates.erase(kh); return fail(BEAGLE_ERROR_GENERAL, "tree-walk scheduler: cannot place this list"); }
            t.key = key;
            it = w4templates.find(kh);
        } else {
            scheduleHits++;
        }
        const Walk4Template& t = it->second;
        reloads += t.reloads; externals += t.externals; phases = std::max(phases, t.phases);
        Plan::Segment sg;
        sg.first = w4table.size();
        sg.W = t.W; sg.entries = t.entries; sg.nslots = t.nslots; sg.tail = t.tail;
        sg.plain = t.plain && !wg; sg.peel = t.peel;
        plan.segments.push_back(sg);
        w4table.resize(sg.first + t.prog.size());
        const uint32_t slotb = wg ? wg_block_bytes(S) : 1024u;
        const uint32_t pbuf = wg ? (uint32_t) K * slotb : (uint32_t) ((size_t) (Ppad / 64) * K);
        const uint32_t ebuf = (uint32_t) K * 64u, mbuf = wg ? (uint32_t) (matrixFloats * 4) : (uint32_t) K * 64u;
        int prevKept = -1;
        w4entryOf.assign(seg.size(), -1);
        for (size_t i = 0; i < t.prog.size(); ++i) {
            const Walk4Template::Entry& te = t.prog[i];
            Walk4Entry& e = w4table[sg.first + i];
            std::memset(&e, 0, sizeof e);
            if (i % (size_t) t.entries == 0) prevKept = -1;
            uint32_t flags = te.flags, mode = SCALE_NONE, keep = 0;
            e.ewrite = (uint32_t) scratchScale * ebuf;
            e.eread = (uint32_t) scratchScale * ebuf;
            e.ewrite = (uint32_t) (scratchScale + (int) (i % (size_t) (wg ? MBAMD_WG_SCRATCH_ROWS : MBAMD_W4_SCRATCH_ROWS))) * ebuf;
            if (wg) {
                e.dst = (uint32_t) nBuffers * pbuf;
                if (te.op >= 0) {
                    const Walk4Op& op = seg[te.op];
                    e.dst = (uint32_t) op.dst * pbuf;
                    if (op.tip1) { e.c1 = (uint32_t) op.c1 * (uint32_t) MBAMD_WG_TW; flags |= MBAMD_W4_TIP1; }
                    else if (te.c1slot == 0xFF) { e.c1 = (uint32_t) op.c1 * pbuf; flags |= MBAMD_WG_MEM1; }
                    else e.c1 = (uint32_t) te.c1slot * slotb;
                    if (op.tip2) { e.c2 = (uint32_t) op.c2 * (uint32_t) MBAMD_WG_TW; flags |= MBAMD_W4_TIP2; }
                    else if (te.c2slot == 0xFF) { e.c2 = (uint32_t) op.c2 * pbuf; flags |= MBAMD_WG_MEM2; }
                    else e.c2 = (uint32_t) te.c2slot * slotb;
                    e.m1 = (uint32_t) op.m1 * mbuf;
                    e.m2 = (uint32_t) op.m2 * mbuf;
                    if (te.dslot != 0xFF) { keep = te.dslot; flags |= MBAMD_W4_KEEP; }
                    if (!op.tip1 && te.c1slot != 0xFF && (int) te.c1slot == prevKept) flags |= MBAMD_WG_PREV1;
                    if (!op.tip2 && te.c2slot != 0xFF && (int) te.c2slot == prevKept) flags |= MBAMD_WG_PREV2;
                    prevKept = te.dslot != 0xFF ? (int) te.dslot : -1;
                    mode = op.scaleWrite >= 0 ? SCALE_WRITE : (op.scaleRead >= 0 ? SCALE_READ : SCALE_NONE);
                    if (op.scaleWrite >= 0) e.ewrite = (uint32_t) op.scaleWrite * ebuf;
                    if (op.scaleRead >= 0) e.eread = (uint32_t) op.scaleRead * ebuf;
                    e.ctl = flags | (mode << 8) | ((uint32_t) segList[te.op] << 10) | (keep << 16);
                } else {
                    e.ctl = (flags & (MBAMD_W4_NOP | MBAMD_W4_BARRIER)) | MBAMD_W4_NOP;
                }
                continue;
            }
            if (te.pfOp[0] >= 0) {
                const Walk4Op& p0 = seg[te.pfOp[0]];
                e.dst = (uint32_t) (te.pfChild[0] == 0 ? p0.c1 : p0.c2) * pbuf;
                e.c1 = (uint32_t) te.pfSlot[0] * 1024u;
                flags |= MBAMD_W4_PF0 | MBAMD_W4_NOP;
                if (te.pfOp[1] >= 0) {
                    const Walk4Op& p1 = seg[te.pfOp[1]];
                    e.c2 = (uint32_t) (te.pfChild[1] == 0 ? p1.c1 : p1.c2) * pbuf;
                    e.m1 = (uint32_t) te.pfSlot[1] * 1024u;
                    flags |= MBAMD_W4_PF1;
                }
            } else if (te.op >= 0) {
                const Walk4Op& op = seg[te.op];
                e.dst = (uint32_t) op.dst * pbuf;
                if (op.tip1) { e.c1 = (uint32_t) op.c1 * 32u; flags |= MBAMD_W4_TIP1; }
                else if (te.c1slot == 0xFE) flags |= MBAMD_W4_FWD1;
                else e.c1 = (uint32_t) te.c1slot * 1024u;
                if (op.tip2) { e.c2 = (uint32_t) op.c2 * 32u; flags |= MBAMD_W4_TIP2; }
                else if (te.c2slot == 0xFE) flags |= MBAMD_W4_FWD2;
                else e.c2 = (uint32_t) te.c2slot * 1024u;
                e.m1 = (uint32_t) op.m1 * mbuf;
                e.m2 = (uint32_t) op.m2 * mbuf;
                if (te.dslot != 0xFF) { keep = te.dslot; flags |= MBAMD_W4_KEEP; }
                mode = op.scaleWrite >= 0 ? SCALE_WRITE : (op.scaleRead >= 0 ? SCALE_READ : SCALE_NONE);
                if (op.scaleWrite >= 0) e.ewrite = (uint32_t) op.scaleWrite * ebuf;
                if (op.scaleRead >= 0) e.eread = (uint32_t) op.scaleRead * ebuf;
                w4entryOf[(size_t) te.op] = (int) (sg.first + i);
                const int subTips = w4subTips[(size_t) te.op];
                if (sg.plain && t.W == 1 && subTips >= 2 && subTips <= unstoredTips()) {
                    constexpr int RO = MBAMD_W4_UNSTORED_TIPS_MAX - 1;
                    const int* const sub = &w4subOps[(size_t) te.op * RO];
                    Plan::Unstored u;
                    u.entry = (int) (sg.first + i); u.dst = op.dst;
                    for (int& x : u.inner) x = -1;
                    bool placed = true;
                    for (int j = 0; j < RO && sub[j] >= 0; ++j) {
                        const Walk4Op& so = seg[(size_t) sub[j]];
                        Walk4Recipe::Op& ro = u.r.op[u.r.nops++];
                        ro.mode = so.scaleWrite >= 0 ? SCALE_WRITE : (so.scaleRead >= 0 ? SCALE_READ : SCALE_NONE);
                        ro.in1 = !so.tip1; ro.in2 = !so.tip2;
                        ro.c1 = so.c1; ro.c2 = so.c2;
                        for (int q = 0; q < j; ++q) {
                            if (ro.in1 && seg[(size_t) sub[q]].dst == so.c1) ro.c1 = q;
                            if (ro.in2 && seg[(size_t) sub[q]].dst == so.c2) ro.c2 = q;
                        }
                        if (sub[j] != te.op) { u.inner[j] = w4entryOf[(size_t) sub[j]]; placed = placed && u.inner[j] >= 0; }
                    }
                    if (placed) plan.unstoredSubtrees.push_back(u);
                }
            }
            if (te.vmwait != 0xFF) flags |= MBAMD_W4_VMWAIT;
            if ((i + 1) % (size_t) t.entries != 0) {
                const Walk4Template::Entry& tn = t.prog[i + 1];
                if (tn.op >= 0 && seg[tn.op].scaleWrite < 0 && seg[tn.op].scaleRead >= 0) flags |= MBAMD_W4_NEXT_READS;
            }
            e.ctl = flags | (mode << 8) | ((uint32_t) (te.vmwait == 0xFF ? 0 : te.vmwait) << 10) | (keep << 16);
            if (sg.plain) {
                if (te.op >= 0) e.ctl |= walk4_kind_of(flags);
                e.eread = (flags & MBAMD_W4_TIP1) ? e.c1 : 0u;
            }
        }
        lastWalkW = t.W; lastWalkSlots = t.nslots; lastWalkEntries = t.entries; lastWalkPhases = t.phases;
        seg.clear();
        segList.clear();
        std::fill(segRead.begin(), segRead.end(), 0);
        std::fill(segWritten.begin(), segWritten.end(), 0);
        std::fill(segScale.begin(), segScale.end(), 0);
        return BEAGLE_SUCCESS;
    };
    for (int o = 0; o < n; ++o) {
        const BeagleOperation& b = ops[o];
        const char* what;
        if (const int crc = checkOperation(b, written, what)) return fail(crc, what);
        Walk4Op w;
        w.dst = b.destinationPartials;
        w.c1 = b.child1Partials; w.c2 = b.child2Partials;
        w.m1 = b.child1TransitionMatrix; w.m2 = b.child2TransitionMatrix;
        const uint8_t tip[2] = {(uint8_t) (tipStates[w.c1] && !written[w.c1]), (uint8_t) (tipStates[w.c2] && !written[w.c2])};
        w.tip1 = tip[0]; w.tip2 = tip[1];
        w.scaleWrite = w.scaleRead = -1;
        if (b.destinationScaleWrite != BEAGLE_OP_NONE) {
            w.scaleWrite = b.destinationScaleWrite;
        } else if (b.destinationScaleRead != BEAGLE_OP_NONE) {
            if (scaleState[b.destinationScaleRead] == 2 && !segScale[b.destinationScaleRead])
                return fail(BEAGLE_ERROR_NO_IMPLEMENTATION, "beagleUpdatePartials: destinationScaleRead names a cumulative buffer");
            w.scaleRead = b.destinationScaleRead;
        }
        bool hazard = segWritten[w.dst] || segRead[w.dst];
        if (perList && o > 0 && listOf[o] != listOf[o - 1]) hazard = true;
        if (w.scaleWrite >= 0 && segScale[w.scaleWrite]) hazard = true;
        if (w.scaleRead >= 0 && segScale[w.scaleRead] == 2) hazard = true;
        if (hazard) {
            int rc = flushSegment();
            if (rc) return rc;
        }
        segWritten[w.dst] = 1;
        if (!tip[0]) segRead[w.c1] = 1;
        if (!tip[1]) segRead[w.c2] = 1;
        if (w.scaleWrite >= 0) segScale[w.scaleWrite] = 2;
        if (w.scaleRead >= 0 && !segScale[w.scaleRead]) segScale[w.scaleRead] = 1;
        written[w.dst] = 1;
        seg.push_back(w);
        segList.push_back(listOf ? listOf[o] : 0);
    }
    int rc = flushSegment();
    if (rc) return rc;
    if (sw.verbose)
        std::fprintf(stderr, "[mbamd] walk plan: %d ops, %zu segment(s), W=%d, %d entries/wave, %d slots/wave, %d phases, %d reloads, %d external children\n",
                     n, plan.segments.size(), lastWalkW, lastWalkEntries, lastWalkSlots, phases, reloads, externals);
    plan.inlineProg.clear();
    const bool inlineForm = !sw.noInlinePrograms && plan.segments.size() == 1 && w4table.size() <= (size_t) MBAMD_W4_INLINE;
    plan.sideFirst = 0; plan.sideCount = 0;
    if (s4 && !sw.storeTipPairs && !sw.noPlainWalk && !inlineForm && plan.segments.size() == 1 && plan.segments[0].plain) {
        for (const Plan::Unstored& u : plan.unstoredSubtrees) w4table[(size_t) u.entry].ctl |= MBAMD_W4_NOSTORE;
        plan.sideFirst = w4table.size();
        for (const Plan::Unstored& u : plan.unstoredSubtrees) {
            if (u.r.nops < 2) continue;
            Walk4Entry side;
            std::memset(&side, 0, sizeof side);
            side.ctl = (uint32_t) u.entry; side.dst = (uint32_t) (u.r.nops - 1);
            side.c1 = (uint32_t) u.inner[0]; side.c2 = (uint32_t) (u.r.nops > 2 ? u.inner[1] : u.inner[0]);
            w4table.push_back(side);
            plan.sideCount++;
        }
    } else {
        plan.unstoredSubtrees.clear();
    }
    if (inlineForm) {
        plan.inlineProg = w4table;
        return BEAGLE_SUCCESS;
    }
    return planTable(plan, w4table.data(), w4table.size() * sizeof(Walk4Entry));
}

inline int Instance::ringCopy(void* dst, const void* src, size_t bytes)
{
    const void* ring = nullptr;
    int rc = stageDirect(src, bytes, &ring);
    if (rc) return rc;
    if (bytes % 16 == 0 && (reinterpret_cast<uintptr_t>(dst) & 15u) == 0) {
        const unsigned n16 = (unsigned) (bytes / 16);
        MBAMD_LAUNCH(k_copy_from_ring, (n16 + 255u) / 256u, 256, 0, stream, static_cast<const copy16_t*>(ring), static_cast<copy16_t*>(dst), n16);
    } else {
        const unsigned n4 = (unsigned) (bytes / 4);
        MBAMD_LAUNCH(k_copy_from_ring4, (n4 + 255u) / 256u, 256, 0, stream, static_cast<const unsigned*>(ring), static_cast<unsigned*>(dst), n4);
    }
    HIP_TRY(hipGetLastError());
    return BEAGLE_SUCCESS;
}

inline bool Instance::recognisePath(const BeagleOperation* ops, int n, int L, bool& forked)
{
    std::vector<char>& written = w4written;
    written.assign((size_t) nBuffers, 0);
    std::vector<char>& named = w4segScale;
    named.assign(scale.size() + 1, 0);
    for (int o = 0; o < n; ++o) {
        const BeagleOperation& b = ops[o];
        const char* what;
        if (checkOperation(b, written, what) != BEAGLE_SUCCESS) return false;
        if (tipStates[b.destinationPartials] || written[b.destinationPartials]) return false;
        written[b.destinationPartials] = 1;
        for (int f : {b.destinationScaleWrite, b.destinationScaleRead})
            if (f >= 0 && f < nScale && named[f] < 3) ++named[f];
    }
    pathSteps.resize((size_t) n);
    forked = false;
    int saved = -1;
    int armStart = 0, arms = 0;
    for (int o = 0; o < n; ++o) {
        const BeagleOperation& b = ops[o];
        PathStep& p = pathSteps[(size_t) o];
        const bool first = o % L == 0;
        const int prev = first ? -1 : ops[o - 1].destinationPartials;
        const bool one = !first && b.child1Partials == prev, two = !first && b.child2Partials == prev;
        if (one && two) return false;
        p.start = !one && !two;
        p.join = false;
        p.arm = 0;
        p.dst = b.destinationPartials;
        p.chain = two ? b.child2Partials : b.child1Partials; p.sib = two ? b.child1Partials : b.child2Partials;
        p.mchain = two ? b.child2TransitionMatrix : b.child1TransitionMatrix; p.msib = two ? b.child1TransitionMatrix : b.child2TransitionMatrix;
        if (p.start) {
            if (!first) {
                if (saved >= 0) return false;
                saved = prev;
                pathSteps[(size_t) armStart].arm = o - armStart;
            }
            armStart = o;
            ++arms;
        } else if (saved >= 0 && p.sib == saved) {
            p.join = true;
            saved = -1;
        }
// ... 58 lines not shown

inline bool Instance::buildPath4(Plan& plan, const BeagleOperation* ops, int n)
{
    if (sw.noPath4 || n < 1 || n > MBAMD_W4_INLINE) return false;
    bool forked;
    if (!recognisePath(ops, n, n, forked) || (forked && sw.noForkPath)) return false;
    const uint32_t pbuf = (uint32_t) ((size_t) (Ppad / 64) * K), mbuf = (uint32_t) K * 64u;
    plan.inlineProg.resize((size_t) n);
    for (int i = 0; i < n; ++i) {
        const PathStep& p = pathSteps[(size_t) i];
        plan.inlineProg[(size_t) i] = pathEntry(p, pbuf, 32u, mbuf, (int) scale.size());
        plan.inlineProg[(size_t) i].ctl |= (uint32_t) p.arm << 16;
    }
    plan.path = true;
    pathPlan(plan, n, forked);
    return true;
}

static inline bool pathg_compiled(int S) { return S == 20 || (S >= 60 && S <= 63); }
inline bool Instance::buildPathG(Plan& plan, const BeagleOperation* ops, int n, const std::vector<int>& starts, int nl)
{
    if (sw.noPathG || !pathg_compiled(S) || nl < 1 || nl > MBAMD_WG_MAXLISTS || n < nl || n % nl != 0) return false;
    const int L = n / nl;
    if (L < 2 || (size_t) n > (size_t) MBAMD_W4_INLINE) return false;
    for (int q = 0; q < nl; ++q) if (starts[(size_t) q] != q * L) return false;
    bool forked;
    if (!recognisePath(ops, n, L, forked) || (forked && sw.noForkPath)) return false;
    for (int o = L; o < n; ++o)
        if (pathSteps[(size_t) o].start != pathSteps[(size_t) (o % L)].start || pathSteps[(size_t) o].join != pathSteps[(size_t) (o % L)].join) return false;
    const uint32_t pbuf = (uint32_t) K * wg_block_bytes(S), mbuf = (uint32_t) (matrixFloats * 4);
    plan.inlineProg.resize((size_t) n);
    for (int o = 0; o < n; ++o) {
        plan.inlineProg[(size_t) o] = pathEntry(pathSteps[(size_t) o], pbuf, (uint32_t) MBAMD_WG_TW, mbuf, (int) scale.size() + (o % L) % MBAMD_WG_SCRATCH_ROWS);
        plan.inlineProg[(size_t) o].ctl |= (uint32_t) (o / L) << 10;
    }
    if (sw.verbose) std::fprintf(stderr, "[mbamd] walk plan: %d list(s) of %d operations each: root-ward paths%s (k_pathg)\n", nl, L, forked ? " that join" : "");
    plan.pathG = true;
    plan.lists = nl;
    pathPlan(plan, L, forked);
    return true;
}

inline Walk4Args Instance::walk4Args() const
{
    Walk4Args a{};
    a.partials = reinterpret_cast<f4*>(arenaPartials);
    a.pstride = geom.pstride;
    a.tips = arenaTips;
    a.tstride = geom.tstride;
    a.exps = arenaExp;
    a.estride = estride;
    a.matrices = matrices;
    a.K = K;
    a.Ppad = Ppad;
    a.nblocks = Ppad / 64;
    return a;
}

inline int Instance::runWalk(const Plan& plan, int32_t* cum)
{
    Walk4ArgsInline ai;
    Walk4Args& a = ai.a;
    a = walk4Args();
    a.cum = cum;
    if (!plan.inlineProg.empty()) std::memcpy(ai.inl, plan.inlineProg.data(), plan.inlineProg.size() * sizeof(Walk4Entry));
    if (plan.path) {
        a.entries = (int) plan.inlineProg.size();
        a.cumFresh = walkCumFresh ? 1 : 0;
        auto kernel = k_path4<Walk4ArgsInline>;
        MBAMD_LAUNCH_BARRIER(kernel, walk4_grid(Ppad / 64, K), 64, path4_lds_bytes((int) plan.inlineProg.size()), stream, ai);
        HIP_TRY(hipGetLastError());
        pendingLaunches += 1;
        return BEAGLE_SUCCESS;
    }
    for (const Plan::Segment& sg : plan.segments) {
        a.entries = sg.entries;
        a.nslots = sg.nslots;
        a.cumFresh = (walkCumFresh && &sg == &plan.segments.front()) ? 1 : 0;
        a.tail = sg.tail;
        bool plainHere = false;
        if (!plan.inlineProg.empty()) {
            auto kernel = k_walk4_t<Walk4ArgsInline>;
            MBAMD_LAUNCH_BARRIER(kernel, walk4_grid(Ppad / 64, K), 64 * sg.W, walk4_lds_bytes(sg.W, sg.nslots), stream, ai);
        } else if (sg.plain && !sw.noPlainWalk) {
            a.prog = reinterpret_cast<const Walk4Entry*>(plan.d_table) + sg.first;
            a.tail = sg.tail + (sg.peel ? 1 : 0);
            auto kernel = k_walk4_t<Walk4Args, true>;
            MBAMD_LAUNCH_BARRIER(kernel, walk4_grid(Ppad / 64, K), 64, walk4_lds_bytes(1, sg.nslots), stream, a);
            plainHere = true;
            if (!plan.unstoredSubtrees.empty()) { const int urc = leaveUnstored(plan); if (urc) return urc; }
        } else {
            a.prog = reinterpret_cast<const Walk4Entry*>(plan.d_table) + sg.first;
            auto kernel = k_walk4_t<Walk4Args>;
            MBAMD_LAUNCH_BARRIER(kernel, walk4_grid(Ppad / 64, K), 64 * sg.W, walk4_lds_bytes(sg.W, sg.nslots), stream, a);
        }
        HIP_TRY(hipGetLastError());
        ++(plainHere ? walksPlain : walksGeneric);
        pendingLaunches += 1;
    }
    return BEAGLE_SUCCESS;
}

inline int Instance::leaveUnstored(const Plan& plan)
{
    if (!d_snap) HIP_TRY(hipMalloc(&d_snap, (size_t) nBuffers * MBAMD_W4_SNAP * K * 16 * sizeof(float)));
    if (snapPlan && snapPlan != &plan) { int rc = flushSnapshot(); if (rc) return rc; }
    for (const Plan::Unstored& u : plan.unstoredSubtrees) {
        if (!unstored[(size_t) u.dst]) ++nUnstored;
        unstored[(size_t) u.dst] = 1;
        recipes[(size_t) u.dst] = u.r;
        ++(u.r.nops > 1 ? leftUnstoredSub : leftUnstored);
    }
    snapPlan = const_cast<Plan*>(&plan);
    return BEAGLE_SUCCESS;
}

inline int Instance::flushSnapshot()
{
    Plan* const plan = snapPlan;
    snapPlan = nullptr;
    if (!plan || plan->segments.size() != 1 || !plan->d_table) return BEAGLE_SUCCESS;
    const Plan::Segment& sg = plan->segments[0];
    plan->lastLaunch = ++launchClock;
    const unsigned nprog = (unsigned) (sg.entries - sg.tail);
    MBAMD_LAUNCH(k_walk4_snapshot, nprog + (unsigned) plan->sideCount, 64, 0, stream, reinterpret_cast<const Walk4Entry*>(plan->d_table) + sg.first,
                 nprog, reinterpret_cast<const Walk4Entry*>(plan->d_table) + plan->sideFirst, (unsigned) ((size_t) (Ppad / 64) * K), (const float*) matrices, d_snap, K);
    HIP_TRY(hipGetLastError());
    return BEAGLE_SUCCESS;
}

inline int Instance::ensureStored(const int* bufs, int n)
{
    if (nUnstored == 0) return BEAGLE_SUCCESS;
    std::vector<int>& list = storeList;
    list.clear();
    for (int i = 0; i < n; ++i) {
        const int b = bufs[i];
        if (b < 0 || b >= nBuffers || unstored[(size_t) b] != 1) continue;
        unstored[(size_t) b] = 2;
        list.push_back(b);
    }
    for (int b : list) unstored[(size_t) b] = 1;
    if (list.empty()) return BEAGLE_SUCCESS;
    int rc = flushSnapshot();
    if (rc) return rc;
    for (int b : list) if (recipes[(size_t) b].nops > 1) return ensureStoredSubtrees();
    const int m = (int) list.size(), entries = (m + 1) / 2 * 2 + 2;
    const uint32_t pbuf = (uint32_t) ((size_t) (Ppad / 64) * K), ebuf = (uint32_t) K * 64u, mbuf = (uint32_t) K * 64u;
    const uint32_t scratch = (uint32_t) scale.size();
    storeProg.resize((size_t) entries);
    for (int i = 0; i < entries; ++i) {
        Walk4Entry& e = storeProg[(size_t) i];
        std::memset(&e, 0, sizeof e);
        e.ctl = MBAMD_W4_NOP;
        e.ewrite = (scratch + (uint32_t) (i % MBAMD_W4_SCRATCH_ROWS)) * ebuf;
        e.eread = scratch * ebuf;
        if (i >= m) continue;
        const uint32_t b = (uint32_t) list[(size_t) i];
        const Recipe& r = recipes[b];
        e.ctl = MBAMD_W4_TIP1 | MBAMD_W4_TIP2 | ((uint32_t) r.op[0].mode << 8);
        e.dst = b * pbuf;
        e.c1 = (uint32_t) r.op[0].c1 * 32u;
        e.c2 = (uint32_t) r.op[0].c2 * 32u;
        e.m1 = ((uint32_t) MBAMD_W4_SNAP * b) * mbuf;
        e.m2 = ((uint32_t) MBAMD_W4_SNAP * b + 1u) * mbuf;
    }
    Walk4ArgsInline ai;
    Walk4Args& a = ai.a;
    a = walk4Args();
    a.matrices = d_snap;
    a.cum = nullptr;
    a.cumFresh = 0;
    a.entries = entries;
    a.nslots = 1;
    a.tail = 2;
    ++launchClock;
    if (entries <= MBAMD_W4_INLINE) {
        std::memcpy(ai.inl, storeProg.data(), (size_t) entries * sizeof(Walk4Entry));
        auto kernel = k_walk4_t<Walk4ArgsInline>;
        MBAMD_LAUNCH_BARRIER(kernel, walk4_grid(Ppad / 64, K), 64, walk4_lds_bytes(1, 1), stream, ai);
    } else {
        const size_t bytes = (size_t) entries * sizeof(Walk4Entry);
        rc = grow(&d_storeProg, &storeProgCap, bytes);
        if (rc) return rc;
        rc = upload(d_storeProg, storeProg.data(), bytes);
        if (rc) return rc;
        a.prog = static_cast<const Walk4Entry*>(d_storeProg);
        auto kernel = k_walk4_t<Walk4Args>;
        MBAMD_LAUNCH_BARRIER(kernel, walk4_grid(Ppad / 64, K), 64, walk4_lds_bytes(1, 1), stream, a);
    }
    HIP_TRY(hipGetLastError());
    for (int b : list) unstored[(size_t) b] = 0;
    nUnstored -= m;
    materialised += m;
    materialiseLaunches += 1;
    return BEAGLE_SUCCESS;
}

inline int Instance::ensureStoredSubtrees()
{
    const std::vector<int>& list = storeList;
    const uint32_t pbuf = (uint32_t) ((size_t) (Ppad / 64) * K), ebuf = (uint32_t) K * 64u, mbuf = (uint32_t) K * 64u;
    const uint32_t scratch = (uint32_t) scale.size();
    storeProg.clear();
    int pairs = 0, subtrees = 0;
    for (int b : list) {
        const Recipe& r = recipes[(size_t) b];
// ... 1301 lines not shown
```

### mrbayes_amd/csrc/mbamd_switches.h

```cpp
#pragma once

#include <cstdlib>
#include <optional>
#include <string>

namespace mbamd {

struct Switches {
    bool stats = false;
    bool apiTrace = false;
    bool verbose = false;
    bool walkTrace = false;
    bool reportDevice = false;
    std::string mpiRank;
    std::optional<int> shard;
    bool forceGeneric = false;
    bool noWalkG = false;
    bool noMfma = false;
    bool mfmaWhole = false;
    bool noDefer = false;
    bool noInlinePrograms = false;
    bool noPlainWalk = false;
    bool storeTipPairs = false;
    std::optional<int> unstoredTips;
    bool noPath4 = false;
    bool noFusePath = false;
    bool noForkPath = false;
    bool noPathG = false;
    std::optional<int> mfmaSerial;
    bool noSpine = false;
    std::optional<int> spineWidth;
    bool noPoll = false;
    std::optional<int> walkWaves;
    std::optional<int> maxLdsSlots;
    std::optional<int> walkSmallPhase;
    std::optional<int> walkPrefetch;
    bool walkSafe = false;
    bool eigen256 = false;
    bool xprodGeneric = false;
    std::optional<int> parsPhaseLimit;
    std::optional<int> parsWaves;
    bool f64NoWalk = false;
    bool f64WalkAlways = false;
    std::optional<int> f64WalkSlots;
    bool f64NoRing = false;
    bool f64NoMatrixQueue = false;
    bool f64MfmaNoLds = false;
    bool f64NoChain = false;
    bool f64NoTipsKernel = false;
};

inline Switches read_switches()
{
    auto on = [](const char* name) { return std::getenv(name) != nullptr; };
    auto num = [](const char* name) -> std::optional<int> {
        const char* e = std::getenv(name);
        return e ? std::optional<int>(std::atoi(e)) : std::nullopt;
    };
    Switches s;
    s.stats = on("MBAMD_STATS"); s.apiTrace = on("MBAMD_API_TRACE"); s.verbose = on("MBAMD_VERBOSE"); s.walkTrace = on("MBAMD_WALK_TRACE");
    s.reportDevice = on("MBAMD_REPORT_DEVICE"); s.shard = num("MBAMD_SHARD");
    if (const char* e = std::getenv("MBAMD_MPI_RANK")) s.mpiRank = e;
    s.forceGeneric = on("MBAMD_FORCE_GENERIC"); s.noWalkG = on("MBAMD_NO_WALKG"); s.noMfma = on("MBAMD_NO_MFMA"); s.mfmaWhole = on("MBAMD_MFMA_WHOLE");
    s.noDefer = on("MBAMD_NO_DEFER"); s.noInlinePrograms = on("MBAMD_NO_INLINE_PROGRAMS"); s.noPath4 = on("MBAMD_NO_PATH4");
    s.noPlainWalk = on("MBAMD_NO_PLAIN_WALK"); s.storeTipPairs = on("MBAMD_STORE_TIP_PAIRS"); s.unstoredTips = num("MBAMD_UNSTORED_TIPS");
    s.noFusePath = on("MBAMD_NO_FUSE_PATH"); s.noForkPath = on("MBAMD_NO_FORK_PATH"); s.noPathG = on("MBAMD_NO_PATHG");
    s.mfmaSerial = num("MBAMD_MFMA_SERIAL"); s.noSpine = on("MBAMD_NO_SPINE"); s.spineWidth = num("MBAMD_SPINE_WIDTH"); s.noPoll = on("MBAMD_NO_POLL");
    s.walkWaves = num("MBAMD_WALK_WAVES"); s.maxLdsSlots = num("MBAMD_MAX_LDS_SLOTS"); s.walkSmallPhase = num("MBAMD_WALK_SMALL_PHASE");
    s.walkPrefetch = num("MBAMD_WALK_PREFETCH"); s.walkSafe = on("MBAMD_WALK_SAFE"); s.eigen256 = on("MBAMD_EIGEN_256");
    s.xprodGeneric = on("MBAMD_XPROD_GENERIC");
    s.parsPhaseLimit = num("MBAMD_PARS_PHASE_LIMIT"); s.parsWaves = num("MBAMD_PARS_WAVES");
    s.f64NoWalk = on("MBAMD_F64_NO_WALK"); s.f64WalkAlways = on("MBAMD_F64_WALK_ALWAYS"); s.f64WalkSlots = num("MBAMD_F64_WALK_SLOTS");
    s.f64NoRing = on("MBAMD_F64_NO_RING"); s.f64NoMatrixQueue = on("MBAMD_F64_NO_MATRIX_QUEUE"); s.f64MfmaNoLds = on("MBAMD_F64_MFMA_NO_LDS");
    s.f64NoChain = on("MBAMD_F64_NO_CHAIN"); s.f64NoTipsKernel = on("MBAMD_F64_NO_TIPS_KERNEL");
    return s;
}

}
```

### mrbayes_amd/csrc/mbamd_walk4.h

```cpp
#include "mbamd_kernels.h"
#ifndef MBAMD_WALK4_H_
#define MBAMD_WALK4_H_

namespace mbamd {

#define MBAMD_W4_NOP      0x01u
#define MBAMD_W4_BARRIER  0x02u
#define MBAMD_W4_PF0      0x04u
#define MBAMD_W4_PF1      0x08u
#define MBAMD_W4_VMWAIT   0x10u
#define MBAMD_W4_TIP1     0x20u
#define MBAMD_W4_TIP2     0x40u
#define MBAMD_W4_KEEP     0x80u
#define MBAMD_W4_FWD1     0x01000000u
#define MBAMD_W4_FWD2     0x02000000u
#define MBAMD_W4_READS      0x00000200u
#define MBAMD_W4_NEXT_READS 0x04000000u
#define MBAMD_W4_NOSTORE  0x20000000u
#define MBAMD_W4_NOSTORE_BIT 29
static_assert(MBAMD_W4_NOSTORE == 1u << MBAMD_W4_NOSTORE_BIT, "the kernel tests the bit by its number");
#define MBAMD_W4_GROUP_FWD2    0x08000000u
#define MBAMD_W4_GROUP_FWD1    0x10000000u
#define MBAMD_W4_GROUP_OTHER   0x40000000u
#define MBAMD_W4_IS_TIP_TIP    0x00000400u
#define MBAMD_W4_IS_TIP_FWD    0x00000800u
#define MBAMD_W4_IS_FWD_TIP    0x00001000u
#define MBAMD_W4_IS_SLOT_FWD   0x00002000u
#define MBAMD_W4_IS_FWD_SLOT   0x00004000u
#define MBAMD_W4_IS_GENERAL    0x00008000u
#define MBAMD_W4_KIND_TIP_TIP  (MBAMD_W4_GROUP_OTHER | MBAMD_W4_IS_TIP_TIP)
#define MBAMD_W4_KIND_TIP_FWD  (MBAMD_W4_GROUP_FWD2 | MBAMD_W4_IS_TIP_FWD)
#define MBAMD_W4_KIND_FWD_TIP  (MBAMD_W4_GROUP_FWD1 | MBAMD_W4_IS_FWD_TIP)
#define MBAMD_W4_KIND_SLOT_FWD (MBAMD_W4_GROUP_FWD2 | MBAMD_W4_IS_SLOT_FWD)
#define MBAMD_W4_KIND_FWD_SLOT (MBAMD_W4_GROUP_FWD1 | MBAMD_W4_IS_FWD_SLOT)
#define MBAMD_W4_KIND_GENERAL  (MBAMD_W4_GROUP_OTHER | MBAMD_W4_IS_GENERAL)
#define MBAMD_W4_KIND_MASK     0x5800FC00u
#define MBAMD_W4_RARE     (MBAMD_W4_NOP | MBAMD_W4_BARRIER | MBAMD_W4_PF0 | MBAMD_W4_VMWAIT | MBAMD_W4_READS | MBAMD_W4_NEXT_READS)
#define MBAMD_W4_SCRATCH_ROWS 32
#define MBAMD_W4_MAXW     8

struct alignas(32) Walk4Entry {
    uint32_t ctl;
    uint32_t dst;
    uint32_t c1;
    uint32_t c2;
    uint32_t m1;
    uint32_t m2;
    uint32_t ewrite;
    uint32_t eread;
};
static_assert(sizeof(Walk4Entry) == 32, "Walk4Entry is 8 dwords");

struct Walk4Args {
    const Walk4Entry* prog;
    int entries;
    int nslots;
    f4* partials;
    unsigned long pstride;
    const uint64_t* tips;
    unsigned tstride;
    int8_t* exps;
    unsigned estride;
    const float* matrices;
    int32_t* cum;
    int cumFresh;
    int K, Ppad, nblocks;
    int tail;
};

#define MBAMD_W4_STAGE 768
__host__ __device__ inline size_t walk4_lds_bytes(int W, int nslots) { return (size_t) W * (MBAMD_W4_STAGE + (size_t) nslots * 1024); }
__host__ __device__ inline unsigned walk4_grid(int nblocks, int K) { return 8u * (unsigned) K * (unsigned) ((nblocks + 7) / 8); }

struct Walk4Planes { uint64_t p[4]; };

}
#include <mbamd_dev_walk4.h>
#include <mbamd_dev_walk4_store.h>
#include <mbamd_dev_walk4_kinds.h>
namespace mbamd {

__host__ __device__ inline unsigned walk4_round_wait(long n)
{
    const unsigned ok[] = {0, 1, 2, 3, 4, 5, 6, 8, 10, 12, 16, 20, 24, 32, 40, 48};
    unsigned r = 0;
    for (unsigned v : ok) if ((long) v <= n) r = v;
    return r;
}

__host__ __device__ inline uint32_t walk4_kind_of(uint32_t flags)
{
    const bool t1 = (flags & MBAMD_W4_TIP1) != 0, t2 = (flags & MBAMD_W4_TIP2) != 0;
    const bool f1 = !t1 && (flags & MBAMD_W4_FWD1) != 0, f2 = !t2 && (flags & MBAMD_W4_FWD2) != 0;
    const bool s1 = !t1 && !f1, s2 = !t2 && !f2;
    if (t1 && t2) return MBAMD_W4_KIND_TIP_TIP;
    if (t1 && f2) return MBAMD_W4_KIND_TIP_FWD;
    if (f1 && t2) return MBAMD_W4_KIND_FWD_TIP;
    if (s1 && f2) return MBAMD_W4_KIND_SLOT_FWD;
    if (f1 && s2) return MBAMD_W4_KIND_FWD_SLOT;
    return MBAMD_W4_KIND_GENERAL;
}
enum { W4K_ANY = 0, W4K_TIP = 1, W4K_FWD = 2, W4K_SLOT = 3 };
template <int V> struct Walk4Kind { static constexpr int value = V; };
struct Walk4Factors { f4 f1, f2; };

template <class T> __device__ __forceinline__ T* walk4_at_kib(T* base, unsigned kib)
{
    return reinterpret_cast<T*>(reinterpret_cast<char*>(base) + ((size_t) kib << 10));
}
template <class T> __device__ __forceinline__ T* walk4_at(T* base, unsigned byteOffset)
{
    return reinterpret_cast<T*>(reinterpret_cast<uintptr_t>(base) + byteOffset);
}

#define MBAMD_W4_INLINE 96
struct Walk4ArgsInline {
    Walk4Args a;
    Walk4Entry inl[MBAMD_W4_INLINE];
};
__device__ __forceinline__ const Walk4Args& walk4_args(const Walk4Args& a) { return a; }
__device__ __forceinline__ const Walk4Args& walk4_args(const Walk4ArgsInline& a) { return a.a; }
__device__ __forceinline__ const Walk4Entry* walk4_program(const Walk4Args& a) { return a.prog; }
}
#include <mbamd_dev_walk4_args.h>
namespace mbamd {

template <class ARGS, bool PLAIN = false>
__global__ void __launch_bounds__(64 * MBAMD_W4_MAXW)
k_walk4_t(ARGS AA)
{
    const Walk4Args& A = walk4_args(AA);
    const unsigned lane = threadIdx.x & 63;
    const int wave = mbd_wave_index();
    char* lds = mbd_dyn_lds<char>();
    const unsigned K = (unsigned) A.K;
    const unsigned xcd = blockIdx.x & 7u, pos = blockIdx.x >> 3;
    const unsigned blk = (pos / K) * 8u + xcd, k = pos % K;
    if (blk >= (unsigned) A.nblocks) return;
    char* const mine = lds + (size_t) wave * (MBAMD_W4_STAGE + (size_t) A.nslots * 1024);
    int* const stage = reinterpret_cast<int*>(mine);
    char* const slots = mine + MBAMD_W4_STAGE + lane * 16;
    f4* const P0 = A.partials + (size_t) blk * A.pstride + (size_t) k * 64;
    const uint64_t* const T0 = A.tips + (size_t) blk * A.tstride;
    int8_t* const E0 = A.exps + (size_t) blk * A.estride + (size_t) k * 64;
    const float* const M0 = A.matrices + (size_t) k * 16;
    const Walk4Lds L = walk4_lds(mine, lane);
#define MBAMD_W4_PREFETCH(SRC, DST) walk4_prefetch(L, walk4_at_kib(P0, SRC), (DST))
#define MBAMD_W4_EXPS(OFF, PARITY) walk4_fetch_exps(L, walk4_at(E0, OFF), lane, (PARITY))

    const Walk4Entry* pp = walk4_program(AA) + (size_t) wave * A.entries;
    const int n = A.entries - A.tail;
    Walk4Entry DA = walk4_load_entry(pp), DB = walk4_load_entry(pp + 1);
    Walk4Mat M1 = walk4_load_matrix(walk4_at(M0, DA.m1));
    Walk4Mat M2 = walk4_load_matrix(walk4_at(M0, DA.m2));
    static_assert(MBAMD_W4_TIP2 == 1u << 6, "the plain loop masks child 2's plane offset with ctl bit 6");
    Walk4Planes T1 = walk4_load_planes(walk4_at(T0, (DA.ctl & MBAMD_W4_TIP1) ? DA.c1 : 0u));
    Walk4Planes T2 = walk4_load_planes(walk4_at(T0, (DA.ctl & MBAMD_W4_TIP2) ? DA.c2 : 0u));
    if constexpr (!PLAIN) { if (DA.ctl & MBAMD_W4_READS) MBAMD_W4_EXPS(DA.eread, 0); }
    int cum_e = 0;
    f4 RA = {0.0f, 0.0f, 0.0f, 0.0f}, RB = RA;

    auto factors = [&](auto k1, auto k2, const Walk4Entry& cur, const f4& prev) {
        constexpr int C1 = decltype(k1)::value, C2 = decltype(k2)::value;
        const unsigned ctl = cur.ctl;
        f4 a, b;
        if constexpr (C1 == W4K_SLOT) a = *reinterpret_cast<const f4*>(slots + cur.c1);
        if constexpr (C2 == W4K_SLOT) b = *reinterpret_cast<const f4*>(slots + cur.c2);
        if constexpr (C1 == W4K_TIP) a = walk4_tip_vector(T1, lane);
        if constexpr (C1 == W4K_FWD) a = prev;
        if constexpr (C1 == W4K_ANY) {
            if (ctl & MBAMD_W4_TIP1) a = walk4_tip_vector(T1, lane);
            else if (ctl & MBAMD_W4_FWD1) a = prev;
            else a = *reinterpret_cast<const f4*>(slots + cur.c1);
        }
        if constexpr (C2 == W4K_TIP) b = walk4_tip_vector(T2, lane);
        if constexpr (C2 == W4K_FWD) b = prev;
        if constexpr (C2 == W4K_ANY) {
            if (ctl & MBAMD_W4_TIP2) b = walk4_tip_vector(T2, lane);
            else if (ctl & MBAMD_W4_FWD2) b = prev;
            else b = *reinterpret_cast<const f4*>(slots + cur.c2);
        }
        Walk4Factors f;
        f.f1 = walk4_matvec(M1, a);
        f.f2 = walk4_matvec(M2, b);
        return f;
    };
    auto step = [&](Walk4Entry& cur, const Walk4Entry& nxt, const Walk4Entry* after, int parity, f4& out, const f4& prev) {
        const unsigned ctl = cur.ctl;
        int er = 0;
        if (!PLAIN && (ctl & MBAMD_W4_RARE)) {
            if (ctl & MBAMD_W4_PF0) {
                MBAMD_W4_PREFETCH(cur.dst, cur.c1);
                if (ctl & MBAMD_W4_PF1) MBAMD_W4_PREFETCH(cur.c2, cur.m1);
            }
            if (ctl & MBAMD_W4_VMWAIT) walk4_wait_vm((ctl >> 10) & 63u);
            if (ctl & MBAMD_W4_BARRIER) walk4_barrier();
            if (ctl & MBAMD_W4_NEXT_READS) MBAMD_W4_EXPS(nxt.eread, parity ^ 1);
            if (ctl & MBAMD_W4_READS) er = stage[64 * parity + lane];
        }
        f4 o = prev;
        Walk4Factors f;
        constexpr Walk4Kind<W4K_ANY> any{};
        if constexpr (PLAIN) {
            constexpr Walk4Kind<W4K_TIP> tip{};
            constexpr Walk4Kind<W4K_FWD> fwd{};
            constexpr Walk4Kind<W4K_SLOT> slot{};
            if (ctl & MBAMD_W4_GROUP_FWD2) {
                if (ctl & MBAMD_W4_IS_TIP_FWD) f = factors(tip, fwd, cur, prev);
                if (ctl & MBAMD_W4_IS_SLOT_FWD) f = factors(slot, fwd, cur, prev);
            }
            if (ctl & MBAMD_W4_GROUP_FWD1) {
                if (ctl & MBAMD_W4_IS_FWD_TIP) f = factors(fwd, tip, cur, prev);
                if (ctl & MBAMD_W4_IS_FWD_SLOT) f = factors(fwd, slot, cur, prev);
            }
            if (ctl & MBAMD_W4_GROUP_OTHER) {
                if (ctl & MBAMD_W4_IS_TIP_TIP) f = factors(tip, tip, cur, prev);
                if (ctl & MBAMD_W4_IS_GENERAL) f = factors(any, any, cur, prev);
            }
        } else {
            if (!(ctl & MBAMD_W4_NOP)) f = factors(any, any, cur, prev);
        }
        if constexpr (PLAIN) o = walk4_product(f.f1, f.f2);
        else if (!(ctl & MBAMD_W4_NOP)) { o.x = f.f1.x * f.f2.x; o.y = f.f1.y * f.f2.y; o.z = f.f1.z * f.f2.z; o.w = f.f1.w * f.f2.w; }
        const unsigned dst = cur.dst, ewrite = cur.ewrite;
        M1 = walk4_load_matrix(walk4_at(M0, nxt.m1));
        M2 = walk4_load_matrix(walk4_at(M0, nxt.m2));
        if constexpr (PLAIN) {
            T1 = walk4_load_planes(walk4_at(T0, nxt.eread));
            T2 = walk4_load_planes(walk4_at(T0, nxt.c2 & (unsigned) ((int) (nxt.ctl << 25) >> 31)));
        } else {
            T1 = walk4_load_planes(walk4_at(T0, (nxt.ctl & MBAMD_W4_TIP1) ? nxt.c1 : 0u));
            T2 = walk4_load_planes(walk4_at(T0, (nxt.ctl & MBAMD_W4_TIP2) ? nxt.c2 : 0u));
        }
        cur = walk4_load_entry(after);
        if (PLAIN || !(ctl & MBAMD_W4_NOP)) {
            const int wm = (int) (ctl << 23) >> 31;
            const int ew = scale_exponent(max4(o)) & wm;
            const int e = ew | er;
            cum_e += ew;
            o.x = scale_pow2(o.x, -e); o.y = scale_pow2(o.y, -e);
            o.z = scale_pow2(o.z, -e); o.w = scale_pow2(o.w, -e);
            if (ctl & MBAMD_W4_KEEP) *reinterpret_cast<f4*>(slots + ((ctl >> 6) & 0x3FC00u)) = o;
            if constexpr (PLAIN) walk4_store_unless(walk4_at_kib(P0, dst), walk4_at(E0, ewrite), lane, o, e, ctl);
            else walk4_store(walk4_at_kib(P0, dst), walk4_at(E0, ewrite), lane, o, e);
        }
        out = o;
    };
    for (int j = 0; j + (PLAIN ? 1 : 0) < n; j += 2) {
        step(DA, DB, pp + 2, 0, RA, RB);
        step(DB, DA, pp + 3, 1, RB, RA);
        pp += 2;
    }
    if constexpr (PLAIN) { if (n & 1) step(DA, DB, pp + 2, 0, RA, RB); }
#undef MBAMD_W4_EXPS
#undef MBAMD_W4_PREFETCH
    if (A.cum != nullptr) {
        const int W = (int) (blockDim.x >> 6);
        if (!PLAIN && W > 1) {
            stage[lane] = cum_e;
            walk4_barrier();
            if (wave != 0) return;
            cum_e = 0;
            for (int w = 0; w < W; ++w)
                cum_e += reinterpret_cast<const int*>(lds + (size_t) w * (MBAMD_W4_STAGE + (size_t) A.nslots * 1024))[lane];
        }
        int32_t* dst = A.cum + (size_t) k * A.Ppad + (size_t) blk * 64 + lane;
        if (A.cumFresh) *dst = cum_e;
        else if (cum_e != 0) *dst += cum_e;
    }
}

#define MBAMD_W4_UNSTORED_TIPS_MAX 4
#define MBAMD_W4_SNAP (2u * (MBAMD_W4_UNSTORED_TIPS_MAX - 1))
__global__ void __launch_bounds__(64)
k_walk4_snapshot(const Walk4Entry* prog, unsigned nprog, const Walk4Entry* side, unsigned kibPerBuffer, const float* matrices, float* snap, int K)
{
    const unsigned n = (unsigned) K * 16u;
    if (blockIdx.x >= nprog) {
        const Walk4Entry* const r = side + (blockIdx.x - nprog);
        float* const dst = snap + ((size_t) (prog[r->ctl].dst / kibPerBuffer) * MBAMD_W4_SNAP + 2u) * n;
        for (unsigned i = threadIdx.x; i < 2u * r->dst * n; i += 64u) {
            const unsigned c = i / n, j = i - c * n;
            const Walk4Entry* const e = prog + (c < 2u ? r->c1 : r->c2);
            dst[i] = matrices[(size_t) (((c & 1u) ? e->m2 : e->m1) >> 2) + j];
        }
        return;
    }
    const Walk4Entry* const e = prog + blockIdx.x;
    if (!(e->ctl & MBAMD_W4_NOSTORE)) return;
    float* const dst = snap + (size_t) (e->dst / kibPerBuffer) * MBAMD_W4_SNAP * n;
    for (unsigned i = threadIdx.x; i < 2u * n; i += 64u) {
        const unsigned c = i / n, j = i - c * n;
        dst[i] = matrices[(size_t) ((c ? e->m2 : e->m1) >> 2) + j];
    }
}

#define MBAMD_P4_START 0x08000000u
#define MBAMD_P4_JOIN  0x10000000u
#if !defined(MBAMD_P4_CHUNK)
#define MBAMD_P4_CHUNK 24
#endif
#define MBAMD_P4_GROUP 4
#define MBAMD_P4_MATRIX_BYTES (MBAMD_P4_CHUNK * 2 * 64)
__device__ __forceinline__ int walk4_path_run(const Walk4Entry* pp, int n, unsigned lane, f4* P0, const uint64_t* T0, int8_t* E0, const float* M0, f4& prev, f4* MS)
{
    constexpr int C = MBAMD_P4_CHUNK;
    static_assert(C % 8 == 0, "eight entries' matrices per vector load");
    int cum_e = 0;
    f4 saved = {0.0f, 0.0f, 0.0f, 0.0f};
    prev = saved;
    for (int arm0 = 0, arm1 = 0; arm0 < n; arm0 = arm1) {
    {
        const Walk4Entry e0 = walk4_entry_from_lds(pp + arm0);
        arm1 = arm0 + (int) ((e0.ctl >> 16) & 0xFFu);
        saved = prev;
        if (e0.ctl & MBAMD_W4_TIP1) prev = walk4_tip_vector(walk4_load_planes(walk4_at(T0, e0.c1)), lane);
        else prev = walk4_at_kib(P0, e0.c1)[lane];
    }
    for (int base = arm0; base < arm1; base += C) {
        const int cnt = arm1 - base < C ? arm1 - base : C;
        const Walk4Entry* const q = pp + base;
        f4 F[C];
        int er[C];
        f4 mq[C / 8];
#pragma unroll
        for (int r = 0; r < C / 8; ++r) {
            const int i = 8 * r + (int) (lane >> 3);
            mq[r] = f4{0.0f, 0.0f, 0.0f, 0.0f};
            if (i < cnt) {
                const Walk4Entry* const ep = q + i;
                const unsigned off = (lane & 4u) ? ep->m2 : ep->m1;
                mq[r] = walk4_load_f4(reinterpret_cast<const f4*>(walk4_at(M0, off)) + (lane & 3u));
            }
        }
#pragma unroll
        for (int i = 0; i < C; ++i) {
            er[i] = 0;
            if (i < cnt) {
                const Walk4Entry e = walk4_entry_from_lds(q + i);
                if (!(e.ctl & (MBAMD_W4_TIP2 | MBAMD_P4_JOIN))) F[i] = walk4_at_kib(P0, e.c2)[lane];
                if (e.ctl & MBAMD_W4_READS) er[i] = walk4_at(E0, e.eread)[lane];
            }
        }
#pragma unroll
        for (int r = 0; r < C / 8; ++r) MS[(size_t) r * 64 + lane] = mq[r];
        walk4_wave_lds_fence();
        constexpr int G = MBAMD_P4_GROUP;
// ... 177 lines not shown
```

### mrbayes_amd/csrc/mbamd_walk4_host.h

```cpp
#ifndef MBAMD_WALK4_HOST_H_
#define MBAMD_WALK4_HOST_H_

#include <algorithm>
#include <functional>
#include <cstdint>
#include <cstring>
#include <queue>
#include <utility>
#include <vector>

#include "mbamd_kernels.h"

namespace mbamd {

struct Walk4Op {
    int dst, c1, c2;
    int m1, m2;
    int scaleWrite, scaleRead;
    uint8_t tip1, tip2;
};

struct Walk4Template {
    struct Entry {
        int op = -1;
        uint8_t flags = 0;
        uint8_t c1slot = 0xFF, c2slot = 0xFF, dslot = 0xFF;
        uint8_t vmwait = 0xFF;
        bool reread = false;
        int pfOp[2] = {-1, -1};
        uint8_t pfChild[2] = {0, 0}, pfSlot[2] = {0, 0};
    };
    std::vector<int> key;
    int W = 1, entries = 0, nslots = 1;
    int tail = 2;
    std::vector<Entry> prog;
    int phases = 1, reloads = 0, externals = 0;
    int evictions = 0;
    bool plain = false, peel = false;
};

struct Walk4Scratch {
    std::vector<int> prod1, prod2, parent, ncons, need, size, phaseOf, waveOf, posOf, order, stack, heapTmp;
    std::vector<char> assigned, cap;
    std::vector<int> binLoad, roots, frontier, slotHolder, lastUse, slotOfVal, freeFrom, memAt, nextOp, pieces, load, dryNodes;
    std::vector<char> fwd;
    std::vector<std::vector<int>> phaseStart;
    std::vector<Walk4Template::Entry> scan;
    std::vector<std::vector<Walk4Template::Entry>> fin;
};

class Walk4Builder {
public:
    int maxW = 1;
    int maxSlots = 8;
    int maxSlots1 = 8;
    int prefetchDistance = 6;
    bool safeWaits = false;
    int smallPhase = 16;
    bool memSlots = true;
    bool alwaysKeep = false;
    bool phasesAreLaunches = false;
    int leadNops = 0, unroll = 2, tailNops = 2;
    bool forward = false;

    bool build(const std::vector<Walk4Op>& ops, Walk4Template& t);

private:
    Walk4Scratch s;
    void suOrder(int root, std::vector<int>& out);
};

inline void Walk4Builder::suOrder(int root, std::vector<int>& out)
{
    std::vector<int>& st = s.stack;
    st.clear();
    st.push_back(root << 1);
    const int ph = s.phaseOf[root];
    while (!st.empty()) {
        const int top = st.back();
        st.pop_back();
        const int o = top >> 1;
        if (top & 1) { out.push_back(o); continue; }
        st.push_back((o << 1) | 1);
        int a = s.prod1[o], b = (s.prod2[o] != s.prod1[o]) ? s.prod2[o] : -1;
        if (a >= 0 && (s.phaseOf[a] != ph || s.parent[a] != o)) a = -1;
        if (b >= 0 && (s.phaseOf[b] != ph || s.parent[b] != o)) b = -1;
        if (a >= 0 && b >= 0 && s.need[b] > s.need[a]) std::swap(a, b);
        if (b >= 0) st.push_back(b << 1);
        if (a >= 0) st.push_back(a << 1);
    }
}

inline bool Walk4Builder::build(const std::vector<Walk4Op>& ops, Walk4Template& t)
{
    const int n = (int) ops.size();
    if (n == 0) return false;
    std::vector<int>&prod1 = s.prod1, &prod2 = s.prod2, &parent = s.parent, &ncons = s.ncons;
    prod1.assign(n, -1); prod2.assign(n, -1); parent.assign(n, -1); ncons.assign(n, 0);
    {
        int maxBuf = 0;
        for (const Walk4Op& o : ops) maxBuf = std::max(maxBuf, std::max(o.dst, std::max(o.tip1 ? 0 : o.c1, o.tip2 ? 0 : o.c2)));
        std::vector<int>& writer = s.heapTmp;
        writer.assign((size_t) maxBuf + 1, -1);
        for (int o = 0; o < n; ++o) {
            if (!ops[o].tip1) prod1[o] = writer[ops[o].c1];
            if (!ops[o].tip2) prod2[o] = writer[ops[o].c2];
            writer[ops[o].dst] = o;
        }
    }
    bool dag = false;
    for (int o = 0; o < n; ++o) {
        const int a = prod1[o], b = (prod2[o] != prod1[o]) ? prod2[o] : -1;
        if (a >= 0) { if (ncons[a]++ > 0) dag = true; else parent[a] = o; }
        if (b >= 0) { if (ncons[b]++ > 0) dag = true; else parent[b] = o; }
    }
    int W = dag ? 1 : std::max(1, std::min(maxW, 8));
    if (n < 2 * smallPhase) W = 1;

    std::vector<int>&phaseOf = s.phaseOf, &waveOf = s.waveOf, &need = s.need, &size = s.size;
    phaseOf.assign(n, -1); waveOf.assign(n, 0); need.assign(n, 1); size.assign(n, 1);
    std::vector<char>& cap = s.cap;
    int nphases = 0;
    std::vector<std::vector<std::vector<int>>> seq;
    int remaining = n;
    std::vector<int>&binLoad = s.binLoad, &roots = s.roots, &frontier = s.frontier;
    while (remaining > 0) {
        const int ph = nphases++;
        seq.emplace_back(std::vector<std::vector<int>>(W));
        for (int o = 0; o < n; ++o) {
            if (phaseOf[o] >= 0) continue;
            int a = prod1[o], b = (prod2[o] != prod1[o]) ? prod2[o] : -1;
            if (a >= 0 && (phaseOf[a] >= 0 || parent[a] != o)) a = -1;
            if (b >= 0 && (phaseOf[b] >= 0 || parent[b] != o)) b = -1;
            const int na = a >= 0 ? need[a] : 0, nb = b >= 0 ? need[b] : 0;
            need[o] = std::max(1, (na == nb) ? na + (na > 0 ? 1 : 0) : std::max(na, nb));
            size[o] = 1 + (a >= 0 ? size[a] : 0) + (b >= 0 ? size[b] : 0);
        }
        roots.clear();
        for (int o = 0; o < n; ++o)
            if (phaseOf[o] < 0 && (parent[o] < 0 || dag)) roots.push_back(o);
        if (dag) {
            for (int o = 0; o < n; ++o) { phaseOf[o] = ph; seq[ph][0].push_back(o); }
            remaining = 0;
            break;
        }
        if (W == 1 || remaining <= smallPhase) {
            int w = 0;
            if (W > 1) {
                binLoad.assign(W, 0);
                for (int o = 0; o < n; ++o) {
                    if (phaseOf[o] >= 0) continue;
                    if (prod1[o] >= 0 && phaseOf[prod1[o]] >= 0) binLoad[waveOf[prod1[o]]]++;
                    if (prod2[o] >= 0 && phaseOf[prod2[o]] >= 0) binLoad[waveOf[prod2[o]]]++;
                }
                w = (int) (std::max_element(binLoad.begin(), binLoad.end()) - binLoad.begin());
            }
            for (int r : roots) phaseOf[r] = ph;
            for (int o = 0; o < n; ++o) if (phaseOf[o] < 0) phaseOf[o] = ph;
            std::sort(roots.begin(), roots.end(), [&](int x, int y) { return size[x] > size[y]; });
            for (int r : roots) suOrder(r, seq[ph][w]);
            for (int o : seq[ph][w]) waveOf[o] = w;
            remaining = 0;
            break;
        }
        cap.assign(n, 0);
        auto cmp = [&](int x, int y) { return size[x] < size[y]; };
        std::priority_queue<int, std::vector<int>, decltype(cmp)> heap(cmp);
        for (int r : roots) heap.push(r);
        const int target = (remaining + W - 1) / W;
        int splits = 0, capSize = 0;
        auto fullestBin = [&](const std::vector<int>& nodes) {
            std::vector<int>&pieces = s.pieces, &load = s.load;
            pieces.clear();
            for (int v : nodes) pieces.push_back(size[v]);
            std::sort(pieces.begin(), pieces.end(), std::greater<int>());
            load.assign(W, 0);
            for (int sz : pieces) *std::min_element(load.begin(), load.end()) += sz;
            return *std::max_element(load.begin(), load.end());
        };
        int bestSplits = 0;
        {
            auto dry = heap;
            std::vector<int>& nodes = s.dryNodes;
            nodes.assign(roots.begin(), roots.end());
            long bestCost = (long) fullestBin(nodes) + 0;
            if ((int) nodes.size() < W) bestCost = 1L << 40;
            int k = 0, capNow = 0;
            while (!dry.empty() && k < 16 * W) {
                const int v = dry.top();
                if (size[v] <= std::max(target / 3, 4)) break;
                dry.pop();
                ++k; ++capNow;
                nodes.erase(std::find(nodes.begin(), nodes.end(), v));
                int a = prod1[v], b = (prod2[v] != prod1[v]) ? prod2[v] : -1;
                if (a >= 0 && phaseOf[a] < 0 && parent[a] == v) { dry.push(a); nodes.push_back(a); }
                if (b >= 0 && phaseOf[b] < 0 && parent[b] == v) { dry.push(b); nodes.push_back(b); }
                if ((int) nodes.size() < W) continue;
                const long cost = (long) fullestBin(nodes) + capNow + 1;
                if (cost < bestCost) { bestCost = cost; bestSplits = k; }
            }
        }
        while (!heap.empty() && splits < bestSplits) {
            const int v = heap.top();
            heap.pop();
            cap[v] = 1; ++capSize; ++splits;
            int a = prod1[v], b = (prod2[v] != prod1[v]) ? prod2[v] : -1;
            if (a >= 0 && phaseOf[a] < 0 && parent[a] == v) heap.push(a);
            if (b >= 0 && phaseOf[b] < 0 && parent[b] == v) heap.push(b);
        }
        frontier.clear();
        while (!heap.empty()) { frontier.push_back(heap.top()); heap.pop(); }
        if (frontier.empty()) {
            for (int o = 0; o < n; ++o) if (phaseOf[o] < 0) { phaseOf[o] = ph; seq[ph][0].push_back(o); }
            remaining = 0;
            break;
        }
        binLoad.assign(W, 0);
        std::vector<int>& st = s.stack;
        for (int r : frontier) {
            const int w = (int) (std::min_element(binLoad.begin(), binLoad.end()) - binLoad.begin());
            binLoad[w] += size[r];
            st.clear();
            st.push_back(r);
            while (!st.empty()) {
                const int o = st.back();
                st.pop_back();
                phaseOf[o] = ph;
                waveOf[o] = w;
                int a = prod1[o], b = (prod2[o] != prod1[o]) ? prod2[o] : -1;
                if (a >= 0 && phaseOf[a] < 0 && parent[a] == o) st.push_back(a);
                if (b >= 0 && phaseOf[b] < 0 && parent[b] == o) st.push_back(b);
            }
        }
        for (int r : frontier) suOrder(r, seq[ph][waveOf[r]]);
        for (int w = 0; w < W; ++w) remaining -= (int) seq[ph][w].size();
        (void) capSize;
    }

    struct Item { int op; uint8_t flags; };
    std::vector<std::vector<Item>> items(W);
    std::vector<int>& posOf = s.posOf;
    posOf.assign(n, -1);
    std::vector<std::vector<int>>& phaseStart = s.phaseStart;
    if ((int) phaseStart.size() < W) phaseStart.resize(W);
    for (int w = 0; w < W; ++w) phaseStart[w].clear();
    for (int ph = 0; ph < nphases; ++ph)
        for (int w = 0; w < W; ++w) {
            if (ph > 0) items[w].push_back(Item{-1, (uint8_t) (MBAMD_W4_NOP | MBAMD_W4_BARRIER)});
            phaseStart[w].push_back((int) items[w].size());
            for (int o : seq[ph][w]) { posOf[o] = (int) items[w].size(); items[w].push_back(Item{o, 0}); }
        }
    size_t longest = 0;
    for (int w = 0; w < W; ++w) longest = std::max(longest, items[w].size());
    t.W = W;
    t.phases = nphases;
    t.reloads = t.externals = t.evictions = 0;
    std::vector<std::vector<Walk4Template::Entry>>& fin = s.fin;
    if ((int) fin.size() < W) fin.resize(W);
    for (int w = 0; w < W; ++w) fin[w].clear();
    std::vector<Walk4Template::Entry>& scan = s.scan;

    int slotsUsed = 1;
    const int S = std::max(memSlots ? 2 : 1, std::min(W == 1 ? std::max(maxSlots, maxSlots1) : maxSlots, 250));
    const int distance = (W == 1 && n <= 128) ? (1 << 20) : prefetchDistance;
    std::vector<int>&slotHolder = s.slotHolder, &lastUse = s.lastUse, &slotOfVal = s.slotOfVal;
    slotHolder.assign(S, 0); lastUse.assign(n, 0); slotOfVal.assign(n, 0);
    struct Mem { int op, child, lo, use; int slot; bool issued; };
    std::vector<Mem> mems;
    std::vector<int>& memAt = s.memAt;
    memAt.clear();
    std::vector<int>& freeFrom = s.freeFrom;
    freeFrom.assign(S, 0);
    for (int w = 0; w < W; ++w) {
        const int L = (int) items[w].size();
        scan.assign((size_t) L, Walk4Template::Entry());
        Walk4Template::Entry* prog = scan.data();
        std::fill(slotHolder.begin(), slotHolder.end(), -1);
        std::fill(freeFrom.begin(), freeFrom.end(), 0);
        for (int j = 0; j < L; ++j) if (items[w][j].op >= 0) { lastUse[items[w][j].op] = -1; slotOfVal[items[w][j].op] = -1; }
        for (int j = 0; j < L; ++j) {
            const int o = items[w][j].op;
            if (o < 0) continue;
            const int pr[2] = {prod1[o], prod2[o]};
            for (int c = 0; c < 2; ++c)
                if (pr[c] >= 0 && waveOf[pr[c]] == w && posOf[pr[c]] < j && (!phasesAreLaunches || phaseOf[pr[c]] == phaseOf[o]))
                    lastUse[pr[c]] = j;
        }
        std::vector<int>& nextOp = s.nextOp;
        std::vector<char>& fwd = s.fwd;
        nextOp.assign((size_t) L + 1, 1 << 30);
        for (int j = L - 1; j >= 0; --j) nextOp[j] = (j + 1 < L && items[w][j + 1].op >= 0) ? j + 1 : nextOp[j + 1];
        if ((int) fwd.size() < n) fwd.resize(n);
        for (int j = 0; j < L; ++j) {
            const int o = items[w][j].op;
            if (o < 0) continue;
            fwd[o] = forward && memSlots && !phasesAreLaunches && ncons[o] == 1 && lastUse[o] == nextOp[j];
        }
        mems.clear();
        auto phaseLo = [&](int j) {
            int lo = 0;
            for (int p : phaseStart[w]) if (p <= j) lo = p;
            return lo;
        };
        for (int j = 0; j < L; ++j) {
            const int o = items[w][j].op;
            if (o < 0) continue;
            const int pr[2] = {prod1[o], prod2[o]};
            const bool tip[2] = {ops[o].tip1 != 0, ops[o].tip2 != 0};
            for (int c = 0; c < 2; ++c) {
                if (tip[c]) continue;
                if (c == 1 && !tip[0] && ops[o].c2 == ops[o].c1) continue;
                if (pr[c] < 0) { if (memSlots) mems.push_back(Mem{o, c, 0, j, -1, false}); t.externals++; }
                else if (waveOf[pr[c]] != w) { if (memSlots) mems.push_back(Mem{o, c, phaseLo(j), j, -1, false}); t.reloads++; }
            }
        }
        auto nextUseOfValue = [&](int v, int from) {
            if (!dag) {
                const int p = parent[v];
                if (p < 0 || waveOf[p] != w) return 1 << 30;
                return posOf[p] >= std::max(from, posOf[v] + 1) ? posOf[p] : (1 << 30);
            }
// ... 139 lines not shown
                    }
                }
                if (sl >= 0) {
                    slotHolder[sl] = o;
                    slotOfVal[o] = sl;
                    e.dslot = (uint8_t) sl;
                    slotsUsed = std::max(slotsUsed, sl + 1);
                } else {
                    t.evictions++;
                    e.reread = true;
                    int uLo = j + 1, uHi = L;
                    if (!dag) { const int p = parent[o]; if (p >= 0 && waveOf[p] == w && posOf[p] >= uLo) { uLo = posOf[p]; uHi = uLo + 1; } else uHi = uLo; }
                    for (int u = uLo; u < uHi; ++u) {
                        const int q = items[w][u].op;
                        if (q < 0) continue;
                        if (prod1[q] == o) { if (memSlots) mems.push_back(Mem{q, 0, j + 1, u, -1, false}); t.reloads++; }
                        if (prod2[q] == o && prod1[q] != o) { if (memSlots) mems.push_back(Mem{q, 1, j + 1, u, -1, false}); t.reloads++; }
                    }
                }
            }
        }
        std::vector<Walk4Template::Entry>& out = fin[w];
        out.clear();
        for (int j = 0; j < L; ++j) {
            Walk4Template::Entry e = prog[j];
            if (e.pfOp[0] >= 0) {
                Walk4Template::Entry pf;
                pf.flags = MBAMD_W4_NOP;
                for (int q = 0; q < 2; ++q) { pf.pfOp[q] = e.pfOp[q]; pf.pfChild[q] = e.pfChild[q]; pf.pfSlot[q] = e.pfSlot[q]; }
                out.push_back(pf);
                e.pfOp[0] = e.pfOp[1] = -1;
            }
            out.push_back(e);
        }
        auto reads = [&](const Walk4Template::Entry& e) { return e.op >= 0 && ops[e.op].scaleRead >= 0 && ops[e.op].scaleWrite < 0; };
        long issued = 0;
        long expSeq = -1;
        if (!out.empty() && reads(out[0])) expSeq = issued++;
        std::vector<long> pfSeq(mems.size(), -1);
        for (size_t j = 0; j < out.size(); ++j) {
            Walk4Template::Entry& e = out[j];
            for (int q = 0; q < 2; ++q)
                if (e.pfOp[q] >= 0) {
                    for (size_t mi = 0; mi < mems.size(); ++mi)
                        if (mems[mi].op == e.pfOp[q] && mems[mi].child == e.pfChild[q] && mems[mi].issued && pfSeq[mi] < 0 &&
                            mems[mi].slot == e.pfSlot[q]) { pfSeq[mi] = issued; break; }
                    ++issued;
                }
            long needed = -1;
            if (e.op >= 0) {
                for (size_t mi = 0; mi < mems.size(); ++mi)
                    if (mems[mi].op == e.op && pfSeq[mi] >= 0) needed = std::max(needed, pfSeq[mi]);
                if (reads(e)) needed = std::max(needed, expSeq);
            }
            if (needed < 0) e.vmwait = 0xFF;
            else e.vmwait = safeWaits ? 0 : (uint8_t) walk4_round_wait(issued - (needed + 1));
            expSeq = -1;
            if (j + 1 < out.size() && reads(out[j + 1])) expSeq = issued++;
            if (e.op >= 0) issued += 2;
        }
    }
    size_t longestFinal = 0;
    for (int w = 0; w < W; ++w) longestFinal = std::max(longestFinal, fin[w].size());
    const int body = (leadNops + (int) longestFinal + unroll - 1) / unroll * unroll;
    const int tail = tailNops;
    const int entries = body + tail;
    t.entries = entries;
    t.tail = tail;
    t.prog.assign((size_t) W * entries, Walk4Template::Entry());
    for (Walk4Template::Entry& e : t.prog) e.flags = MBAMD_W4_NOP;
    for (int w = 0; w < W; ++w) std::copy(fin[w].begin(), fin[w].end(), t.prog.begin() + (size_t) w * entries + leadNops);
    t.nslots = slotsUsed;
    t.plain = t.peel = false;
    if (memSlots && W == 1 && leadNops == 0 && unroll == 2 && tail == 2) {
        bool plain = true;
        for (const Walk4Template::Entry& e : fin[0])
            if (e.op < 0 || e.flags != 0 || e.pfOp[0] >= 0 || e.vmwait != 0xFF || (ops[e.op].scaleRead >= 0 && ops[e.op].scaleWrite < 0)) plain = false;
        t.plain = plain;
        t.peel = plain && (int) fin[0].size() == body - 1;
    }
    return true;
}

}
#endif
```

Before: 102,600.

## Split plain tree walk across multiple waves per workgroup with shared LDS slots

```diff
diff --git a/include/libhmsbeagle/beagle.h b/include/libhmsbeagle/beagle.h
--- a/include/libhmsbeagle/beagle.h
+++ b/include/libhmsbeagle/beagle.h
@@ -248,6 +248,7 @@
 BEAGLE_DLLEXPORT int mbamdGetKernelTiming(int instance, double* outMilliseconds, long* outLaunches, int reset);
 BEAGLE_DLLEXPORT int mbamdGetListCounts(int instance, long* out6);
 BEAGLE_DLLEXPORT int mbamdGetWalkCounts(int instance, long* out2);
+BEAGLE_DLLEXPORT int mbamdGetPlainWaveCounts(int instance, long* out8);
 BEAGLE_DLLEXPORT int mbamdGetRecomputeCounts(int instance, long* out3);
 BEAGLE_DLLEXPORT int mbamdGetSubtreeRecomputeCounts(int instance, long* out3);
 BEAGLE_DLLEXPORT int mbamdGetStepTiming(int instance, double* outMilliseconds, long* outSteps, int reset);
diff --git a/mrbayes_amd/beagle.py b/mrbayes_amd/beagle.py
--- a/mrbayes_amd/beagle.py
+++ b/mrbayes_amd/beagle.py
@@ -61,7 +61,7 @@
     "beagleGetScaleFactors", "beagleCalculateRootLogLikelihoods", "beagleCalculateEdgeLogLikelihoods",
     "beagleGetSiteLogLikelihoods", "beagleGetSiteDerivatives", "beagleUpdatePrePartials", "beagleSetDifferentialMatrix",
     "beagleCalculateEdgeDerivatives", "beagleCalculateCrossProductDerivative", "mbamdSynchronize", "mbamdGetLastError", "mbamdKernelTiming",
-    "mbamdGetKernelTiming", "mbamdGetListCounts", "mbamdGetWalkCounts", "mbamdGetRecomputeCounts", "mbamdGetSubtreeRecomputeCounts", "mbamdGetStepTiming", "mbamdUpdateFinalPartials", "mbamdGetScaledPartials", "mbamdSetKernelPath", "mbamdSetDeferredResult", "mbamdFetchLogLikelihood", "mbamdReduceLogLikelihood", "mbamdGetResourcePciBusId", "mbamdGetInstanceDevices",
+    "mbamdGetKernelTiming", "mbamdGetListCounts", "mbamdGetWalkCounts", "mbamdGetPlainWaveCounts", "mbamdGetRecomputeCounts", "mbamdGetSubtreeRecomputeCounts", "mbamdGetStepTiming", "mbamdUpdateFinalPartials", "mbamdGetScaledPartials", "mbamdSetKernelPath", "mbamdSetDeferredResult", "mbamdFetchLogLikelihood", "mbamdReduceLogLikelihood", "mbamdGetResourcePciBusId", "mbamdGetInstanceDevices",
     "mbamdGetScaleExponents", "mbamdGetChildCount", "mbamdSetRateMatrices", "mbamdSetRateMatricesFrom",
     "beagleGetBenchmarkedResourceList", "beagleSetCPUThreadCount", "beagleSetPatternPartitions",
     "beagleSetCategoryRatesWithIndex", "beagleUpdateTransitionMatricesWithMultipleModels", "beagleUpdatePartialsByPartition",
@@ -149,6 +149,7 @@
         L.mbamdGetKernelTiming.argtypes = [C.c_int, _dp, C.POINTER(C.c_long), C.c_int]
         L.mbamdGetListCounts.argtypes = [C.c_int, C.POINTER(C.c_long)]
         L.mbamdGetWalkCounts.argtypes = [C.c_int, C.POINTER(C.c_long)]
+        L.mbamdGetPlainWaveCounts.argtypes = [C.c_int, C.POINTER(C.c_long)]
         L.mbamdGetRecomputeCounts.argtypes = [C.c_int, C.POINTER(C.c_long)]
         L.mbamdGetSubtreeRecomputeCounts.argtypes = [C.c_int, C.POINTER(C.c_long)]
         L.mbamdGetStepTiming.argtypes = [C.c_int, _dp, C.POINTER(C.c_long), C.c_int]
@@ -518,6 +519,11 @@
         self._chk(self.lib.mbamdGetWalkCounts(self.id, out), "mbamdGetWalkCounts")
         return tuple(int(v) for v in out)
 
+    def get_plain_wave_counts(self):
+        out = (C.c_long * 8)()
+        self._chk(self.lib.mbamdGetPlainWaveCounts(self.id, out), "mbamdGetPlainWaveCounts")
+        return tuple(int(v) for v in out)
+
     def get_recompute_counts(self):
         out = (C.c_long * 3)()
         self._chk(self.lib.mbamdGetRecomputeCounts(self.id, out), "mbamdGetRecomputeCounts")
diff --git a/mrbayes_amd/csrc/device/mbamd_dev_walk4_waves.h b/mrbayes_amd/csrc/device/mbamd_dev_walk4_waves.h
--- /dev/null
+++ b/mrbayes_amd/csrc/device/mbamd_dev_walk4_waves.h
@@ -0,0 +1,12 @@
+#ifndef MBAMD_DEV_WALK4_WAVES_H_
+#define MBAMD_DEV_WALK4_WAVES_H_
+namespace mbamd {
+__device__ __forceinline__ void walk4_meet()
+{
+    asm volatile("s_waitcnt lgkmcnt(0)" ::: "memory");
+    __builtin_amdgcn_s_barrier();
+    asm volatile("" ::: "memory");
+}
+__device__ __forceinline__ unsigned walk4_load_word(const uint32_t* p) { return *reinterpret_cast<const MBAMD_AS_CONST uint32_t*>((uintptr_t) p); }
+}
+#endif
diff --git a/mrbayes_amd/csrc/mbamd_engine.cpp b/mrbayes_amd/csrc/mbamd_engine.cpp
--- a/mrbayes_amd/csrc/mbamd_engine.cpp
+++ b/mrbayes_amd/csrc/mbamd_engine.cpp
@@ -1034,6 +1034,14 @@
     in->walkCounts(out2);
     return BEAGLE_SUCCESS;
 }
+int mbamdGetPlainWaveCounts(int instance, long* out8)
+{
+    GET_INSTANCE_NOFLUSH(instance);
+    if (!out8) return fail(BEAGLE_ERROR_OUT_OF_RANGE, "mbamdGetPlainWaveCounts: null output");
+    for (int w = 0; w < MBAMD_W4_MAXW; ++w) out8[w] = 0;
+    if (h->f64) return BEAGLE_SUCCESS;
+    EACH_ENGINE(false, (c->plainWaveCounts(out8), BEAGLE_SUCCESS));
+}
 int mbamdGetRecomputeCounts(int instance, long* out3)
 {
     GET_INSTANCE_NOFLUSH(instance);
diff --git a/mrbayes_amd/csrc/mbamd_f32.h b/mrbayes_amd/csrc/mbamd_f32.h
--- a/mrbayes_amd/csrc/mbamd_f32.h
+++ b/mrbayes_amd/csrc/mbamd_f32.h
@@ -71,6 +71,7 @@
     struct Segment {
         size_t first; int W, entries, nslots, tail = 2;
         bool plain = false, peel = false;
+        bool waves = false;
     };
     std::vector<Segment> segments;
     std::vector<Walk4Entry> inlineProg;
@@ -154,6 +155,7 @@
     int stepTiming(double* ms, long* steps, int reset);
     void listCounts(long out6[6]) const { const long c[6] = {listsTotal, listsPath, forkedPaths, fusedPaths, listsWalked, opsWalked}; std::copy(c, c + 6, out6); }
     void walkCounts(long out2[2]) const { out2[0] = walksPlain; out2[1] = walksGeneric; }
+    void plainWaveCounts(long out[MBAMD_W4_MAXW]) const { for (int w = 0; w < MBAMD_W4_MAXW; ++w) out[w] += walksPlainByW[w]; }
     int walkTrace(long long* out, int maxSteps, int* outSteps, int* outWaves);
     void recomputeCounts(long out3[3]) const { out3[0] += leftUnstored; out3[1] += materialised; out3[2] += materialiseLaunches; }
     void subtreeRecomputeCounts(long out3[3]) const { out3[0] += leftUnstoredSub; out3[1] += materialisedSub; out3[2] += materialiseLaunchesSub; }
@@ -180,7 +182,7 @@
     unsigned estride = 0;
     std::vector<int32_t*> wideScale;
     std::vector<char> scaleState;
-    int lastWalkW = 0, lastWalkSlots = 0, lastWalkEntries = 0, lastWalkPhases = 0;
+    int lastWalkW = 0, lastWalkSlots = 0, lastWalkEntries = 0, lastWalkPhases = 0, lastWalkCrossing = 0;
     bool walkCumFresh = false;
     typedef Walk4Recipe Recipe;
     std::vector<char> unstored;
@@ -416,6 +418,7 @@
     uint64_t planClock = 0;
     int layoutEpoch = 0;
     long planHits = 0, planMisses = 0, fusedPaths = 0, heldPaths = 0, forkedPaths = 0, listsTotal = 0, listsPath = 0, opsWalked = 0, listsWalked = 0;
+    long walksPlainByW[MBAMD_W4_MAXW] = {};
     long walksPlain = 0, walksGeneric = 0;
 
     int grow(void** p, size_t* cap, size_t bytes) { return grow_device(stream, p, cap, bytes, std::max(bytes, *cap * 2)); }
@@ -704,6 +707,16 @@
     (void) hipStreamDestroy(stream);
 }
 
+#define MBAMD_W4_PLAIN_WAVES_PER_CU 32
+#define MBAMD_W4_PLAIN_MAXW 4
+static inline double walk4_entry_us(double wavesPerCU)
+{
+    static const double x[] = {4.9, 9.8, 12.2, 14.7, 19.6, 24.4}, y[] = {0.354, 0.395, 0.428, 0.485, 0.542, 0.747};
+    if (wavesPerCU <= x[0]) return y[0];
+    int i = 1;
+    while (i < 5 && wavesPerCU > x[i]) ++i;
+    return y[i - 1] + (y[i] - y[i - 1]) * (wavesPerCU - x[i - 1]) / (x[i] - x[i - 1]);
+}
 inline int Instance::configureWalk()
 {
     int numCU = 256;
@@ -712,6 +725,7 @@
     const int maxLds = 160 * 1024;
     if (s4 && (hipFuncSetAttribute((const void*) k_walk4_t<Walk4Args>, hipFuncAttributeMaxDynamicSharedMemorySize, maxLds) != hipSuccess ||
                hipFuncSetAttribute((const void*) k_walk4_t<Walk4Args, true>, hipFuncAttributeMaxDynamicSharedMemorySize, maxLds) != hipSuccess ||
+               hipFuncSetAttribute((const void*) k_walk4_t<Walk4Args, true, true>, hipFuncAttributeMaxDynamicSharedMemorySize, maxLds) != hipSuccess ||
                hipFuncSetAttribute((const void*) k_walk4_t<Walk4ArgsInline>, hipFuncAttributeMaxDynamicSharedMemorySize, maxLds) != hipSuccess))
         (void) hipGetLastError();
     if (wg) {
@@ -748,6 +762,22 @@
     w4.forward = true;
     w4.safeWaits = sw.walkSafe;
     if (sw.walkSmallPhase) w4.smallPhase = std::max(1, *sw.walkSmallPhase);
+    {
+        const double wpc = (double) wgs / numCU;
+        double bestTime = walk4_entry_us(wpc);
+        w4.plainWaves = 1;
+        for (int w = 2; w <= MBAMD_W4_PLAIN_MAXW; ++w) {
+            w4.plainShare[w] = (int) (1024.0 * 0.95 * walk4_entry_us(wpc) / walk4_entry_us(wpc * w));
+            if (perCU * w > MBAMD_W4_PLAIN_WAVES_PER_CU) continue;
+            const double tw = walk4_entry_us(wpc * w) / w;
+            if (tw < bestTime) { bestTime = tw; w4.plainWaves = w; }
+        }
+        w4.plainDescend = !sw.walkWaves;
+    }
+    if (sw.walkWaves) w4.plainWaves = W;
+    if (sw.noPlainWalk) w4.plainWaves = 0;
+    w4.plainSlots = std::min(250, sw.maxLdsSlots ? slots : (ldsPerWG - ldsPerWG / 16) / 1024);
+    if (sw.walkPlainMinOps) w4.plainMinOps = std::max(1, *sw.walkPlainMinOps);
     if (sw.verbose) std::fprintf(stderr, "[mbamd] tree walk: %ld workgroups (%d per CU), up to %d waves x %d slots\n", wgs, perCU, W, slots);
     return BEAGLE_SUCCESS;
 }
@@ -1586,6 +1616,7 @@
         key.reserve(seg.size() * 3 + 4);
         key.push_back((int) seg.size()); key.push_back(w4.maxW); key.push_back(w4.maxSlots + 256 * w4.maxSlots1);
         key.push_back(w4.prefetchDistance * 2 + (w4.safeWaits ? 1 : 0));
+        key.push_back(w4.plainWaves + 16 * w4.plainSlots); key.push_back(w4.plainMinOps + 64 * w4.plainShare[std::max(2, std::min(8, w4.plainWaves))] + (w4.plainDescend ? 1 << 20 : 0));
         {
             std::vector<int>& writer = w4writer;
             constexpr int RO = MBAMD_W4_UNSTORED_TIPS_MAX - 1;
@@ -1638,7 +1669,7 @@
         Plan::Segment sg;
         sg.first = w4table.size();
         sg.W = t.W; sg.entries = t.entries; sg.nslots = t.nslots; sg.tail = t.tail;
-        sg.plain = t.plain && !wg; sg.peel = t.peel;
+        sg.plain = t.plain && !wg; sg.peel = t.peel; sg.waves = sg.plain && t.waves;
         plan.segments.push_back(sg);
         w4table.resize(sg.first + t.prog.size());
         const uint32_t slotb = wg ? wg_block_bytes(S) : 1024u;
@@ -1709,7 +1740,7 @@
                 if (op.scaleRead >= 0) e.eread = (uint32_t) op.scaleRead * ebuf;
                 w4entryOf[(size_t) te.op] = (int) (sg.first + i);
                 const int subTips = w4subTips[(size_t) te.op];
-                if (sg.plain && t.W == 1 && subTips >= 2 && subTips <= unstoredTips()) {
+                if (sg.plain && subTips >= 2 && subTips <= unstoredTips()) {
                     constexpr int RO = MBAMD_W4_UNSTORED_TIPS_MAX - 1;
                     const int* const sub = &w4subOps[(size_t) te.op * RO];
                     Plan::Unstored u;
@@ -1742,7 +1773,15 @@
                 e.eread = (flags & MBAMD_W4_TIP1) ? e.c1 : 0u;
             }
         }
-        lastWalkW = t.W; lastWalkSlots = t.nslots; lastWalkEntries = t.entries; lastWalkPhases = t.phases;
+        if (sg.waves) {
+            const size_t at = w4table.size();
+            w4table.resize(at + walk4_waves_table_entries(t.W, t.phases));
+            std::memset(&w4table[at], 0, (w4table.size() - at) * sizeof(Walk4Entry));
+            uint32_t* const tab = reinterpret_cast<uint32_t*>(&w4table[at]);
+            tab[0] = (uint32_t) t.phases;
+            for (size_t q = 0; q < t.phaseCount.size(); ++q) tab[1 + q] = (uint32_t) t.phaseCount[q];
+        }
+        lastWalkW = t.W; lastWalkSlots = t.nslots; lastWalkEntries = t.entries; lastWalkPhases = t.phases; lastWalkCrossing = t.crossing;
         seg.clear();
         segList.clear();
         std::fill(segRead.begin(), segRead.end(), 0);
@@ -1788,10 +1827,11 @@
     int rc = flushSegment();
     if (rc) return rc;
     if (sw.verbose)
-        std::fprintf(stderr, "[mbamd] walk plan: %d ops, %zu segment(s), W=%d, %d entries/wave, %d slots/wave, %d phases, %d reloads, %d external children\n",
-                     n, plan.segments.size(), lastWalkW, lastWalkEntries, lastWalkSlots, phases, reloads, externals);
+        std::fprintf(stderr, "[mbamd] walk plan: %d ops, %zu segment(s), W=%d, %d entries/wave, %d slots/%s, %d phases, %d reloads, %d external children, %d values cross waves in LDS%s\n",
+                     n, plan.segments.size(), lastWalkW, lastWalkEntries, lastWalkSlots, plan.segments.back().waves ? "workgroup" : "wave", phases, reloads, externals,
+                     lastWalkCrossing, plan.segments.back().plain ? " (plain)" : "");
     plan.inlineProg.clear();
-    const bool inlineForm = !sw.noInlinePrograms && plan.segments.size() == 1 && w4table.size() <= (size_t) MBAMD_W4_INLINE;
+    const bool inlineForm = !sw.noInlinePrograms && plan.segments.size() == 1 && w4table.size() <= (size_t) MBAMD_W4_INLINE && !plan.segments[0].waves;
     plan.sideFirst = 0; plan.sideCount = 0;
     if (s4 && !sw.storeTipPairs && !sw.noPlainWalk && !inlineForm && plan.segments.size() == 1 && plan.segments[0].plain) {
         for (const Plan::Unstored& u : plan.unstoredSubtrees) w4table[(size_t) u.entry].ctl |= MBAMD_W4_NOSTORE;
@@ -2016,6 +2056,12 @@
         if (!plan.inlineProg.empty()) {
             auto kernel = k_walk4_t<Walk4ArgsInline>;
             MBAMD_LAUNCH_BARRIER(kernel, walk4_grid(Ppad / 64, K), 64 * sg.W, walk4_lds_bytes(sg.W, sg.nslots), stream, ai);
+        } else if (sg.waves) {
+            a.prog = reinterpret_cast<const Walk4Entry*>(plan.d_table) + sg.first;
+            auto kernel = k_walk4_t<Walk4Args, true, true>;
+            MBAMD_LAUNCH_BARRIER(kernel, walk4_grid(Ppad / 64, K), 64 * sg.W, walk4_waves_lds_bytes(sg.W, sg.nslots), stream, a);
+            plainHere = true;
+            if (!plan.unstoredSubtrees.empty()) { const int urc = leaveUnstored(plan); if (urc) return urc; }
         } else if (sg.plain && !sw.noPlainWalk) {
             a.prog = reinterpret_cast<const Walk4Entry*>(plan.d_table) + sg.first;
             a.tail = sg.tail + (sg.peel ? 1 : 0);
@@ -2030,6 +2076,7 @@
         }
         HIP_TRY(hipGetLastError());
         ++(plainHere ? walksPlain : walksGeneric);
+        if (plainHere) ++walksPlainByW[(sg.waves ? sg.W : 1) - 1];
         pendingLaunches += 1;
     }
     return BEAGLE_SUCCESS;
@@ -2056,7 +2103,7 @@
     if (!plan || plan->segments.size() != 1 || !plan->d_table) return BEAGLE_SUCCESS;
     const Plan::Segment& sg = plan->segments[0];
     plan->lastLaunch = ++launchClock;
-    const unsigned nprog = (unsigned) (sg.entries - sg.tail);
+    const unsigned nprog = sg.waves ? (unsigned) (sg.W * sg.entries) : (unsigned) (sg.entries - sg.tail);
     MBAMD_LAUNCH(k_walk4_snapshot, nprog + (unsigned) plan->sideCount, 64, 0, stream, reinterpret_cast<const Walk4Entry*>(plan->d_table) + sg.first,
                  nprog, reinterpret_cast<const Walk4Entry*>(plan->d_table) + plan->sideFirst, (unsigned) ((size_t) (Ppad / 64) * K), (const float*) matrices, d_snap, K);
     HIP_TRY(hipGetLastError());
diff --git a/mrbayes_amd/csrc/mbamd_switches.h b/mrbayes_amd/csrc/mbamd_switches.h
--- a/mrbayes_amd/csrc/mbamd_switches.h
+++ b/mrbayes_amd/csrc/mbamd_switches.h
@@ -34,6 +34,7 @@
     std::optional<int> walkWaves;
     std::optional<int> maxLdsSlots;
     std::optional<int> walkSmallPhase;
+    std::optional<int> walkPlainMinOps;
     std::optional<int> walkPrefetch;
     bool walkSafe = false;
     bool eigen256 = false;
@@ -67,6 +68,7 @@
     s.noFusePath = on("MBAMD_NO_FUSE_PATH"); s.noForkPath = on("MBAMD_NO_FORK_PATH"); s.noPathG = on("MBAMD_NO_PATHG");
     s.mfmaSerial = num("MBAMD_MFMA_SERIAL"); s.noSpine = on("MBAMD_NO_SPINE"); s.spineWidth = num("MBAMD_SPINE_WIDTH"); s.noPoll = on("MBAMD_NO_POLL");
     s.walkWaves = num("MBAMD_WALK_WAVES"); s.maxLdsSlots = num("MBAMD_MAX_LDS_SLOTS"); s.walkSmallPhase = num("MBAMD_WALK_SMALL_PHASE");
+    s.walkPlainMinOps = num("MBAMD_WALK_PLAIN_MIN_OPS");
     s.walkPrefetch = num("MBAMD_WALK_PREFETCH"); s.walkSafe = on("MBAMD_WALK_SAFE"); s.eigen256 = on("MBAMD_EIGEN_256");
     s.xprodGeneric = on("MBAMD_XPROD_GENERIC");
     s.parsPhaseLimit = num("MBAMD_PARS_PHASE_LIMIT"); s.parsWaves = num("MBAMD_PARS_WAVES");
diff --git a/mrbayes_amd/csrc/mbamd_walk4.h b/mrbayes_amd/csrc/mbamd_walk4.h
--- a/mrbayes_amd/csrc/mbamd_walk4.h
+++ b/mrbayes_amd/csrc/mbamd_walk4.h
@@ -70,6 +70,8 @@
 
 #define MBAMD_W4_STAGE 768
 __host__ __device__ inline size_t walk4_lds_bytes(int W, int nslots) { return (size_t) W * (MBAMD_W4_STAGE + (size_t) nslots * 1024); }
+__host__ __device__ inline size_t walk4_waves_lds_bytes(int W, int nslots) { return (size_t) nslots * 1024 > (size_t) W * 256 ? (size_t) nslots * 1024 : (size_t) W * 256; }
+__host__ __device__ inline size_t walk4_waves_table_entries(int W, int phases) { return ((size_t) phases * W + 1 + 7) / 8; }
 __host__ __device__ inline unsigned walk4_grid(int nblocks, int K) { return 8u * (unsigned) K * (unsigned) ((nblocks + 7) / 8); }
 
 struct Walk4Planes { uint64_t p[4]; };
@@ -78,6 +80,7 @@
 #include <mbamd_dev_walk4.h>
 #include <mbamd_dev_walk4_store.h>
 #include <mbamd_dev_walk4_kinds.h>
+#include <mbamd_dev_walk4_waves.h>
 namespace mbamd {
 
 __host__ __device__ inline unsigned walk4_round_wait(long n)
@@ -125,7 +128,7 @@
 #include <mbamd_dev_walk4_args.h>
 namespace mbamd {
 
-template <class ARGS, bool PLAIN = false>
+template <class ARGS, bool PLAIN = false, bool WAVES = false>
 __global__ void __launch_bounds__(64 * MBAMD_W4_MAXW)
 k_walk4_t(ARGS AA)
 {
@@ -137,9 +140,10 @@
     const unsigned xcd = blockIdx.x & 7u, pos = blockIdx.x >> 3;
     const unsigned blk = (pos / K) * 8u + xcd, k = pos % K;
     if (blk >= (unsigned) A.nblocks) return;
-    char* const mine = lds + (size_t) wave * (MBAMD_W4_STAGE + (size_t) A.nslots * 1024);
-    int* const stage = reinterpret_cast<int*>(mine);
-    char* const slots = mine + MBAMD_W4_STAGE + lane * 16;
+    static_assert(!WAVES || PLAIN, "several waves on the plain loop, or the generic kernel");
+    char* const mine = WAVES ? lds : lds + (size_t) wave * (MBAMD_W4_STAGE + (size_t) A.nslots * 1024);
+    int* const stage = reinterpret_cast<int*>(WAVES ? lds + (size_t) wave * 256 : mine);
+    char* const slots = mine + (WAVES ? 0 : MBAMD_W4_STAGE) + lane * 16;
     f4* const P0 = A.partials + (size_t) blk * A.pstride + (size_t) k * 64;
     const uint64_t* const T0 = A.tips + (size_t) blk * A.tstride;
     int8_t* const E0 = A.exps + (size_t) blk * A.estride + (size_t) k * 64;
@@ -246,23 +250,51 @@
         }
         out = o;
     };
-    for (int j = 0; j + (PLAIN ? 1 : 0) < n; j += 2) {
-        step(DA, DB, pp + 2, 0, RA, RB);
-        step(DB, DA, pp + 3, 1, RB, RA);
-        pp += 2;
-    }
-    if constexpr (PLAIN) { if (n & 1) step(DA, DB, pp + 2, 0, RA, RB); }
+    if constexpr (WAVES) {
+        (void) n;
+        const int W = (int) (blockDim.x >> 6);
+        const uint32_t* const tab = reinterpret_cast<const uint32_t*>(walk4_program(AA) + (size_t) W * A.entries);
+        const int phases = (int) walk4_load_word(tab);
+        const Walk4Entry* base = pp;
+        for (int ph = 0; ph < phases; ++ph) {
+            const int np = (int) walk4_load_word(tab + 1 + ph * W + wave);
+            if (ph > 0) {
+                walk4_meet();
+                pp = base;
+                DA = walk4_load_entry(pp); DB = walk4_load_entry(pp + 1);
+                M1 = walk4_load_matrix(walk4_at(M0, DA.m1));
+                M2 = walk4_load_matrix(walk4_at(M0, DA.m2));
+                T1 = walk4_load_planes(walk4_at(T0, DA.eread));
+                T2 = walk4_load_planes(walk4_at(T0, (DA.ctl & MBAMD_W4_TIP2) ? DA.c2 : 0u));
+            }
+            for (int j = 0; j + 1 < np; j += 2) {
+                step(DA, DB, pp + 2, 0, RA, RB);
+                step(DB, DA, pp + 3, 1, RB, RA);
+                pp += 2;
+            }
+            if (np & 1) step(DA, DB, pp + 2, 0, RA, RB);
+            base += np;
+        }
+    } else {
+        for (int j = 0; j + (PLAIN ? 1 : 0) < n; j += 2) {
+            step(DA, DB, pp + 2, 0, RA, RB);
+            step(DB, DA, pp + 3, 1, RB, RA);
+            pp += 2;
+        }
+        if constexpr (PLAIN) { if (n & 1) step(DA, DB, pp + 2, 0, RA, RB); }
+    }
 #undef MBAMD_W4_EXPS
 #undef MBAMD_W4_PREFETCH
     if (A.cum != nullptr) {
         const int W = (int) (blockDim.x >> 6);
-        if (!PLAIN && W > 1) {
+        if ((!PLAIN || WAVES) && W > 1) {
+            if constexpr (WAVES) walk4_meet();
             stage[lane] = cum_e;
-            walk4_barrier();
+            if constexpr (WAVES) walk4_meet(); else walk4_barrier();
             if (wave != 0) return;
             cum_e = 0;
             for (int w = 0; w < W; ++w)
-                cum_e += reinterpret_cast<const int*>(lds + (size_t) w * (MBAMD_W4_STAGE + (size_t) A.nslots * 1024))[lane];
+                cum_e += reinterpret_cast<const int*>(lds + (size_t) w * (WAVES ? (size_t) 256 : MBAMD_W4_STAGE + (size_t) A.nslots * 1024))[lane];
         }
         int32_t* dst = A.cum + (size_t) k * A.Ppad + (size_t) blk * 64 + lane;
         if (A.cumFresh) *dst = cum_e;
diff --git a/mrbayes_amd/csrc/mbamd_walk4_host.h b/mrbayes_amd/csrc/mbamd_walk4_host.h
--- a/mrbayes_amd/csrc/mbamd_walk4_host.h
+++ b/mrbayes_amd/csrc/mbamd_walk4_host.h
@@ -37,6 +37,9 @@
     int phases = 1, reloads = 0, externals = 0;
     int evictions = 0;
     bool plain = false, peel = false;
+    bool waves = false;
+    std::vector<int> phaseCount;
+    int crossing = 0;
 };
 
 struct Walk4Scratch {
@@ -62,12 +65,17 @@
     bool phasesAreLaunches = false;
     int leadNops = 0, unroll = 2, tailNops = 2;
     bool forward = false;
+    int plainWaves = 0, plainSlots = 0, plainMinOps = 32;
+    int plainShare[9] = {1024, 1024, 1024, 1024, 1024, 1024, 1024, 1024, 1024};
+    bool plainDescend = false;
 
     bool build(const std::vector<Walk4Op>& ops, Walk4Template& t);
 
 private:
     Walk4Scratch s;
     void suOrder(int root, std::vector<int>& out);
+    int forceSplits = -1, splitsMade = 0;
+    bool placePlainWaves(const std::vector<Walk4Op>& ops, Walk4Template& t, const std::vector<std::vector<std::vector<int>>>& seq, int W);
 };
 
 inline void Walk4Builder::suOrder(int root, std::vector<int>& out)
@@ -115,7 +123,14 @@
         if (b >= 0) { if (ncons[b]++ > 0) dag = true; else parent[b] = o; }
     }
     int W = dag ? 1 : std::max(1, std::min(maxW, 8));
+    bool tryPlain = memSlots && forward && !dag && plainWaves > 1 && n >= plainMinOps * plainWaves && leadNops == 0 && unroll == 2 && tailNops == 2;
+    for (int o = 0; o < n && tryPlain; ++o)
+        tryPlain = (ops[o].tip1 || prod1[o] >= 0) && (ops[o].tip2 || prod2[o] >= 0) && !(ops[o].scaleRead >= 0 && ops[o].scaleWrite < 0);
+    if (tryPlain) W = std::min(plainWaves, 8);
     if (n < 2 * smallPhase) W = 1;
+    tryPlain = tryPlain && W > 1;
+    t.waves = false; t.phaseCount.clear(); t.crossing = 0;
+    splitsMade = 0;
 
     std::vector<int>&phaseOf = s.phaseOf, &waveOf = s.waveOf, &need = s.need, &size = s.size;
     phaseOf.assign(n, -1); waveOf.assign(n, 0); need.assign(n, 1); size.assign(n, 1);
@@ -200,6 +215,7 @@
                 if (cost < bestCost) { bestCost = cost; bestSplits = k; }
             }
         }
+        if (tryPlain && forceSplits >= 0 && ph == 0) bestSplits = forceSplits;
         while (!heap.empty() && splits < bestSplits) {
             const int v = heap.top();
             heap.pop();
@@ -214,6 +230,12 @@
             for (int o = 0; o < n; ++o) if (phaseOf[o] < 0) { phaseOf[o] = ph; seq[ph][0].push_back(o); }
             remaining = 0;
             break;
+        }
+        if (tryPlain) {
+            std::vector<int>& big = s.pieces;
+            big.clear();
+            for (int r : frontier) if ((long) size[r] * 16 > (long) remaining) big.push_back(r);
+            if ((int) big.size() >= 2) frontier.assign(big.begin(), big.end());
         }
         binLoad.assign(W, 0);
         std::vector<int>& st = s.stack;
@@ -232,11 +254,48 @@
                 if (b >= 0 && phaseOf[b] < 0 && parent[b] == o) st.push_back(b);
             }
         }
+        if (tryPlain) {
+            splitsMade = std::max(splitsMade, splits);
+            for (int o = 0; o < n; ++o) {
+                if (!cap[o] || phaseOf[o] >= 0) continue;
+                int w = -1;
+                bool same = true;
+                for (const int c : {prod1[o], prod2[o]}) {
+                    if (c < 0) continue;
+                    if (phaseOf[c] != ph || (w >= 0 && waveOf[c] != w)) same = false;
+                    else w = waveOf[c];
+                }
+                if (same && w >= 0) { phaseOf[o] = ph; waveOf[o] = w; }
+            }
+            frontier.clear();
+            for (int o = 0; o < n; ++o)
+                if (phaseOf[o] == ph && (parent[o] < 0 || phaseOf[parent[o]] != ph)) frontier.push_back(o);
+            std::stable_sort(frontier.begin(), frontier.end(), [&](int x, int y) { return need[x] != need[y] ? need[x] > need[y] : size[x] > size[y]; });
+        }
         for (int r : frontier) suOrder(r, seq[ph][waveOf[r]]);
         for (int w = 0; w < W; ++w) remaining -= (int) seq[ph][w].size();
         (void) capSize;
     }
 
+    if (tryPlain) {
+        if (placePlainWaves(ops, t, seq, W)) return true;
+        if (forceSplits >= 0) return false;
+        {
+            Walk4Template best, cand;
+            bool have = false;
+            for (int k = splitsMade - 1; k >= W - 1; --k) {
+                forceSplits = k;
+                if (build(ops, cand) && cand.waves && (!have || cand.entries < best.entries)) { best = cand; have = true; }
+            }
+            forceSplits = -1;
+            if (have) { t = best; return true; }
+        }
+        const int keep = plainWaves;
+        plainWaves = plainDescend && W > 2 ? W - 1 : 0;
+        const bool ok = build(ops, t);
+        plainWaves = keep;
+        return ok;
+    }
     struct Item { int op; uint8_t flags; };
     std::vector<std::vector<Item>> items(W);
     std::vector<int>& posOf = s.posOf;
@@ -542,5 +601,91 @@
     return true;
 }
 
+inline bool Walk4Builder::placePlainWaves(const std::vector<Walk4Op>& ops, Walk4Template& t, const std::vector<std::vector<std::vector<int>>>& seq, int W)
+{
+    const int n = (int) ops.size(), nphases = (int) seq.size();
+    const int S = std::min(plainSlots, 250);
+    if (S < 1) return false;
+    {
+        size_t longest = 0;
+        for (int w = 0; w < W; ++w) {
+            size_t mine = 0;
+            for (const std::vector<std::vector<int>>& phase : seq) mine += phase[(size_t) w].size();
+            longest = std::max(longest, mine);
+        }
+        if (longest >= (size_t) n || longest * 1024 > (size_t) n * (size_t) plainShare[W]) return false;
+    }
+    const std::vector<int>&prod1 = s.prod1, &prod2 = s.prod2, &parent = s.parent, &phaseOf = s.phaseOf, &waveOf = s.waveOf;
+    std::vector<int> owner((size_t) S, -1), holds((size_t) S, -1), slotOf((size_t) n, -1);
+    std::vector<char> inRegs((size_t) n, 0);
+    std::vector<std::vector<Walk4Template::Entry>>& fin = s.fin;
+    if ((int) fin.size() < W) fin.resize(W);
+    for (int w = 0; w < W; ++w) fin[w].clear();
+    int used = 1, crossing = 0;
+    t.phaseCount.assign((size_t) nphases * W, 0);
+    for (int ph = 0; ph < nphases; ++ph) {
+        for (int q = 0; q < S; ++q) {
+            owner[q] = -1;
+            if (holds[q] >= 0) { const int p = parent[holds[q]]; owner[q] = phaseOf[p] == ph ? waveOf[p] : -2; }
+        }
+        for (int w = 0; w < W; ++w) {
+            const std::vector<int>& run = seq[ph][w];
+            t.phaseCount[(size_t) ph * W + w] = (int) run.size();
+            for (size_t i = 0; i < run.size(); ++i) {
+                const int o = run[i];
+                Walk4Template::Entry e;
+                e.op = o;
+                const int pr[2] = {prod1[o], prod2[o]};
+                const bool tip[2] = {ops[o].tip1 != 0, ops[o].tip2 != 0};
+                const bool twice = !tip[0] && !tip[1] && ops[o].c1 == ops[o].c2;
+                uint8_t* cslot[2] = {&e.c1slot, &e.c2slot};
+                for (int c = 0; c < 2; ++c) {
+                    if (tip[c]) continue;
+                    if (c == 1 && twice) { e.c2slot = e.c1slot; continue; }
+                    const int v = pr[c];
+                    if (v < 0) return false;
+                    if (inRegs[v]) { *cslot[c] = 0xFE; continue; }
+                    if (slotOf[v] < 0 || owner[slotOf[v]] != w) return false;
+                    *cslot[c] = (uint8_t) slotOf[v];
+                }
+                for (int c = 0; c < (twice ? 1 : 2); ++c)
+                    if (!tip[c] && *cslot[c] != 0xFE) { holds[*cslot[c]] = -1; slotOf[pr[c]] = -1; }
+                const int p = parent[o];
+                if (p >= 0) {
+                    if (phaseOf[p] < ph || (phaseOf[p] == ph && waveOf[p] != w)) return false;
+                    if (phaseOf[p] == ph && i + 1 < run.size() && run[i + 1] == p) {
+                        inRegs[o] = 1;
+                    } else {
+                        int sl = -1;
+                        for (int q = 0; q < S && sl < 0; ++q) if (holds[q] < 0 && owner[q] == w) sl = q;
+                        for (int q = 0; q < S && sl < 0; ++q) if (holds[q] < 0 && owner[q] == -1) sl = q;
+                        if (sl < 0) return false;
+                        owner[sl] = w; holds[sl] = o; slotOf[o] = sl;
+                        e.dslot = (uint8_t) sl;
+                        used = std::max(used, sl + 1);
+                        if (waveOf[p] != w) ++crossing;
+                    }
+                }
+                fin[w].push_back(e);
+            }
+        }
+    }
+    size_t longest = 0;
+    for (int w = 0; w < W; ++w) longest = std::max(longest, fin[w].size());
+    t.W = W;
+    t.phases = nphases;
+    t.reloads = t.externals = t.evictions = 0;
+    t.tail = 2;
+    t.entries = (int) longest + t.tail;
+    t.prog.assign((size_t) W * t.entries, Walk4Template::Entry());
+    for (Walk4Template::Entry& e : t.prog) e.flags = MBAMD_W4_NOP;
+    for (int w = 0; w < W; ++w) std::copy(fin[w].begin(), fin[w].end(), t.prog.begin() + (size_t) w * t.entries);
+    t.nslots = used;
+    t.plain = t.waves = true;
+    t.peel = false;
+    t.crossing = crossing;
+    return true;
+}
+
 }
 #endif
```

Result: faster. 113,600, median of 6 (+10.7%).
